# bbc/turingcodec

Hardware: AMD Instinct MI355X
Metric: encoded fps (havoc hot path, primitive-batch throughput: one picture's primitive calls per frame as whole-frame batches; (higher is better)
Workload: dtype u8; 1 GPU; 1920x1080 8-bit 4:2:0 random-access QP32 speed=medium B-frame, MEASURED call mix of the reference encoder on this clip generator (profiles/r04_reference_call_mi; calls_per_frame=3944815, launches_per_frame=49, pictures_in_flight=2, parallelism=single GPU

## Files before the change

include/havoc_mi355x.h:

```cpp
#ifndef HAVOC_MI355X_H
#define HAVOC_MI355X_H

#include <stddef.h>
#include <stdint.h>

#ifdef __cplusplus
extern "C" {
#endif

#define HAVOC_MI355X_EINVAL (-10001)
#define HAVOC_MI355X_ENODEV (-10002)
#define HAVOC_MI355X_EDEVICE (-10003)

typedef struct havoc_mi355x_ctx havoc_mi355x_ctx;

#define HAVOC_MI355X_NEW_STREAM ((void *)(intptr_t)-1)
int havoc_mi355x_create(havoc_mi355x_ctx **ctx, int device, void *stream);
void havoc_mi355x_destroy(havoc_mi355x_ctx *ctx);
int havoc_mi355x_set_stream(havoc_mi355x_ctx *ctx, void *stream);
int havoc_mi355x_sync(havoc_mi355x_ctx *ctx);
int havoc_mi355x_sync_spin(havoc_mi355x_ctx *ctx);
const char *havoc_mi355x_last_error(void);
const char *havoc_mi355x_version(void);
int havoc_mi355x_device_info(havoc_mi355x_ctx *ctx, int64_t info[8]);
// ... 92 lines not shown
typedef struct {
    int32_t dst_off, src_off;
    int32_t n;
    int32_t scale, shift, offset;
    int32_t reserved[2];
} havoc_mi355x_quant_job;


int havoc_mi355x_pad_block(havoc_mi355x_ctx *ctx, int S, void *d_plane, int64_t origin_off, int width, int height,
                           intptr_t stride, int pad, int top, int bottom, int left, int right);

int havoc_mi355x_deblock(havoc_mi355x_ctx *ctx, int S, int bitDepth, void *d_luma, intptr_t stride_luma, void *d_cb, void *d_cr, intptr_t stride_chroma,
                         int width, int height, const int8_t *d_block_data, const uint8_t *d_block_bs, int tc_offset_div2, int beta_offset_div2,
                         int cb_qp_offset, int cr_qp_offset);

typedef struct {
    int16_t mv[2][2];
    int8_t dpb_index[2];
    uint8_t flags;
    int8_t qp_y;
    uint8_t tu_log2;
    uint8_t reserved[3];
} havoc_mi355x_cell;
enum {
    HAVOC_CELL_INTRA = 1,
    HAVOC_CELL_CODED = 2,
    HAVOC_CELL_NO_FILTER = 4,
    HAVOC_CELL_PU_LEFT = 8,
    HAVOC_CELL_PU_TOP = 16
};
int havoc_mi355x_derive_bs(havoc_mi355x_ctx *ctx, const havoc_mi355x_cell *d_cells, intptr_t cells_stride, int width, int height, int8_t *d_block_data,
                           uint8_t *d_block_bs);

typedef struct havoc_mi355x_picture havoc_mi355x_picture;
int havoc_mi355x_picture_create(havoc_mi355x_ctx *ctx, int S, int bit_depth, int width, int height, int pad, int alignment,
                                havoc_mi355x_picture **pic);
void havoc_mi355x_picture_destroy(havoc_mi355x_ctx *ctx, havoc_mi355x_picture *pic);
int havoc_mi355x_picture_plane(havoc_mi355x_picture *pic, int cIdx, void **d_base, int64_t *origin_off, intptr_t *stride, int *width, int *height,
                               int *pad);
int havoc_mi355x_picture_upload_yuv(havoc_mi355x_ctx *ctx, havoc_mi355x_picture *pic, const void *h_yuv, int src_S, int shift, int pad_after);
int havoc_mi355x_picture_upload_plane(havoc_mi355x_ctx *ctx, havoc_mi355x_picture *pic, int cIdx, const void *h_origin, intptr_t h_stride,
                                      int with_padding);
int havoc_mi355x_picture_download_plane(havoc_mi355x_ctx *ctx, havoc_mi355x_picture *pic, int cIdx, void *h_origin, intptr_t h_stride,
                                        int with_padding);
int havoc_mi355x_picture_pad(havoc_mi355x_ctx *ctx, havoc_mi355x_picture *pic);
int havoc_mi355x_picture_phase_planes(havoc_mi355x_ctx *ctx, havoc_mi355x_picture *pic, void **d_planes, intptr_t *plane_elems, int64_t *luma_first);


int havoc_mi355x_sad(havoc_mi355x_ctx *ctx, int S, const void *d_src, intptr_t stride_src, const void *d_ref,
                     intptr_t stride_ref, const havoc_mi355x_pair_job *d_jobs, int njobs, int32_t *d_out);
int havoc_mi355x_sad4(havoc_mi355x_ctx *ctx, int S, const void *d_src, intptr_t stride_src, const void *d_ref,
                      intptr_t stride_ref, const havoc_mi355x_sad4_job *d_jobs, int njobs, int32_t *d_out);
typedef struct {
    int32_t first_job;
    int32_t count;
    int32_t box_off, box_w, box_h;
    int32_t reserved[3];
} havoc_mi355x_sad4_run;
int havoc_mi355x_sad4_runs(havoc_mi355x_ctx *ctx, int S, const void *d_src, intptr_t stride_src, const void *d_ref,
                           intptr_t stride_ref, const havoc_mi355x_sad4_job *d_jobs, int njobs,
                           const havoc_mi355x_sad4_run *d_runs, int nruns, int32_t *d_out);
int havoc_mi355x_sad4_make_runs(const havoc_mi355x_sad4_job *jobs, int njobs, int max_run, intptr_t stride_ref, int S, havoc_mi355x_sad4_run *runs);
int havoc_mi355x_sad_surface(havoc_mi355x_ctx *ctx, int S, int range, int max_w, int max_h, const void *d_src,
                             intptr_t stride_src, const void *d_ref, intptr_t stride_ref,
                             const havoc_mi355x_surface_job *d_jobs, int njobs, int32_t *d_out);
int havoc_mi355x_ssd(havoc_mi355x_ctx *ctx, int S, const void *d_a, intptr_t stride_a, const void *d_b,
                     intptr_t stride_b, const havoc_mi355x_pair_job *d_jobs, int njobs, uint32_t *d_out);
int havoc_mi355x_satd(havoc_mi355x_ctx *ctx, int S, int max_w, int max_h, const void *d_a, intptr_t stride_a, const void *d_b,
                      intptr_t stride_b, const havoc_mi355x_pair_job *d_jobs, int njobs, int32_t *d_out);
int havoc_mi355x_satd_multi(havoc_mi355x_ctx *ctx, int S, int max_w, int max_h, const void *d_a, intptr_t stride_a,
                            const void *d_b, intptr_t stride_b, const havoc_mi355x_satd_multi_job *d_jobs, int njobs,
                            int32_t *d_out);
int havoc_mi355x_ssd_linear(havoc_mi355x_ctx *ctx, const uint8_t *d_a, const uint8_t *d_b, int size, int32_t *d_out);


int havoc_mi355x_pred_uni(havoc_mi355x_ctx *ctx, int S, int taps, int bitDepth, int max_w, int max_h, void *d_dst, intptr_t stride_dst,
                          const void *d_ref, intptr_t stride_ref, const havoc_mi355x_pred_uni_job *d_jobs, int njobs);
int havoc_mi355x_pred_bi(havoc_mi355x_ctx *ctx, int S, int taps, int bitDepth, int max_w, int max_h, void *d_dst, intptr_t stride_dst,
                         const void *d_ref, intptr_t stride_ref, const havoc_mi355x_pred_bi_job *d_jobs, int njobs);
int havoc_mi355x_pred_uni_classes(havoc_mi355x_ctx *ctx, int S, int taps, int bitDepth, void *d_dst, intptr_t stride_dst, const void *d_ref,
                                  intptr_t stride_ref, const havoc_mi355x_pred_uni_job *d_jobs, const int32_t count[4]);
int havoc_mi355x_pred_bi_classes(havoc_mi355x_ctx *ctx, int S, int taps, int bitDepth, void *d_dst, intptr_t stride_dst, const void *d_ref,
                                 intptr_t stride_ref, const havoc_mi355x_pred_bi_job *d_jobs, const int32_t count[4]);
int havoc_mi355x_subtract_bi(havoc_mi355x_ctx *ctx, int S, int bitDepth, void *d_dst, intptr_t stride_dst,
                             const void *d_pred, intptr_t stride_pred, const void *d_src, intptr_t stride_src,
                             const havoc_mi355x_subtract_bi_job *d_jobs, int njobs);

int havoc_mi355x_interp_planes(havoc_mi355x_ctx *ctx, int S, int bitDepth, void *d_planes, intptr_t plane_elems, const void *d_ref,
                               intptr_t stride, int x0, int y0, int width, int height);

int havoc_mi355x_subpel_satd(havoc_mi355x_ctx *ctx, int S, int taps, int bitDepth, int max_w, int max_h, const void *d_src,
                             intptr_t stride_src, const void *d_ref, intptr_t stride_ref, const havoc_mi355x_pred_uni_job *d_jobs,
                             int njobs, int32_t *d_cost);


int havoc_mi355x_intra(havoc_mi355x_ctx *ctx, int S, int bitDepth, int log2TrafoSize, void *d_dst, intptr_t stride_dst,
                       const void *d_neighbours, const havoc_mi355x_intra_job *d_jobs, int njobs);

typedef struct {
    int32_t src_off;
    int32_t nb_off;
    int32_t nbf_off;
    uint32_t filt_lo;
    uint32_t filt_hi;
    int32_t edge;
    int32_t reserved[2];
} havoc_mi355x_intra_search_job;
int havoc_mi355x_intra_satd35(havoc_mi355x_ctx *ctx, int S, int bitDepth, int log2TrafoSize, const void *d_src, intptr_t stride_src,
                              const void *d_neighbours, const havoc_mi355x_intra_search_job *d_jobs, int njobs, int32_t *d_cost);


int havoc_mi355x_residual(havoc_mi355x_ctx *ctx, int S, int16_t *d_res, intptr_t stride_res, const int32_t *d_res_off,
                          const void *d_src, intptr_t stride_src, const void *d_pred, intptr_t stride_pred,
                          const havoc_mi355x_pair_job *d_jobs, int njobs);
int havoc_mi355x_transform(havoc_mi355x_ctx *ctx, int bitDepth, int trType, int log2TrafoSize, int16_t *d_coeffs,
                           const int16_t *d_res, intptr_t stride_res, const havoc_mi355x_tu_job *d_jobs, int njobs);
int havoc_mi355x_inverse_transform(havoc_mi355x_ctx *ctx, int bitDepth, int trType, int log2TrafoSize, int16_t *d_res,
                                   const int16_t *d_coeffs, const havoc_mi355x_tu_job *d_jobs, int njobs);
int havoc_mi355x_inverse_transform_add(havoc_mi355x_ctx *ctx, int S, int bitDepth, int trType, int log2TrafoSize,
                                       void *d_dst, intptr_t stride_dst, const void *d_pred, intptr_t stride_pred,
                                       const int16_t *d_coeffs, const havoc_mi355x_tu_job *d_jobs, int njobs);
typedef struct {
    int32_t coef_off;
    int32_t src_off;
    int32_t pred_off;
    int32_t rec_off;
} havoc_mi355x_tu_fused_job;
int havoc_mi355x_tu_forward(havoc_mi355x_ctx *ctx, int S, int bitDepth, int trType, int log2TrafoSize, int16_t *d_coeffs, const void *d_src,
                            intptr_t stride_src, const void *d_pred, intptr_t stride_pred, const havoc_mi355x_tu_fused_job *d_jobs, int njobs);
int havoc_mi355x_intra_measure(havoc_mi355x_ctx *ctx, int S, int bitDepth, int log2TrafoSize, int16_t *d_coeffs, int16_t *d_coeffs_dct, int32_t *d_satd, void *d_rec0,
                               uint32_t *d_ssd0, const void *d_src, intptr_t stride_src, const void *d_pred, intptr_t stride_pred, const havoc_mi355x_tu_fused_job *d_jobs,
                               int njobs, int with_satd);
int havoc_mi355x_tu_reconstruct(havoc_mi355x_ctx *ctx, int S, int bitDepth, int trType, int log2TrafoSize, int scale, int shift, void *d_rec,
                                intptr_t stride_rec, const void *d_pred, intptr_t stride_pred, const void *d_src, intptr_t stride_src,
                                const int16_t *d_levels, const havoc_mi355x_tu_fused_job *d_jobs, int njobs, uint32_t *d_ssd);

int havoc_mi355x_level_stats(havoc_mi355x_ctx *ctx, const int16_t *d_levels, const int32_t *d_jobs, int njobs, int32_t *d_out);

int havoc_mi355x_quantize(havoc_mi355x_ctx *ctx, int16_t *d_dst, const int16_t *d_src,
                          const havoc_mi355x_quant_job *d_jobs, int njobs, int32_t *d_cbf);
int havoc_mi355x_quantize_inverse(havoc_mi355x_ctx *ctx, int16_t *d_dst, const int16_t *d_src,
                                  const havoc_mi355x_quant_job *d_jobs, int njobs);
int havoc_mi355x_quantize_reconstruct(havoc_mi355x_ctx *ctx, int log2TrafoSize, uint8_t *d_rec, intptr_t stride_rec,
                                      const uint8_t *d_pred, intptr_t stride_pred, const int16_t *d_res,
                                      const havoc_mi355x_tu_job *d_jobs, int njobs);

typedef struct {
    int32_t src_off, rec_off;
    int32_t w, h;
} havoc_mi355x_sao_stats_job;
int havoc_mi355x_sao_stats(havoc_mi355x_ctx *ctx, int S, int bitDepth, const void *d_src, intptr_t stride_src, const void *d_rec, intptr_t stride_rec,
                           const havoc_mi355x_sao_stats_job *d_jobs, int njobs, int64_t *d_out);
typedef struct {
    int32_t src_u, src_v;
    int32_t rec_u, rec_v;
    int32_t w, h;
    int32_t reserved[2];
} havoc_mi355x_sao_chroma_job;
int havoc_mi355x_sao_band_chroma(havoc_mi355x_ctx *ctx, int S, int bitDepth, const void *d_src, intptr_t stride_src, const void *d_rec, intptr_t stride_rec,
                                 const havoc_mi355x_sao_chroma_job *d_jobs, int njobs, int64_t *d_out);
typedef struct {
    int32_t dst_off, src_off, w, h;
    int32_t type, eo_class;
    int16_t offsets[32];
    int32_t reserved[2];
} havoc_mi355x_sao_job;
// ... 439 lines not shown
```

turingcodec_amd/csrc/api.hip:

```cpp
#include "common.h"
#include "launch.h"

#include <cstdio>
#include <cstring>
#include <initializer_list>

using namespace havoc_gpu;

static_assert(sizeof(havoc_mi355x_pair_job) == 16, "job ABI");
static_assert(sizeof(havoc_mi355x_sad4_job) == 32, "job ABI");
static_assert(sizeof(havoc_mi355x_surface_job) == 32, "job ABI");
static_assert(sizeof(havoc_mi355x_satd_multi_job) == 80, "job ABI");
static_assert(sizeof(havoc_mi355x_pred_uni_job) == 32, "job ABI");
static_assert(sizeof(havoc_mi355x_pred_bi_job) == 48, "job ABI");
static_assert(sizeof(havoc_mi355x_subtract_bi_job) == 32, "job ABI");
static_assert(sizeof(havoc_mi355x_intra_job) == 32, "job ABI");
static_assert(sizeof(havoc_mi355x_tu_job) == 16, "job ABI");
static_assert(sizeof(havoc_mi355x_intra_search_job) == 32, "job ABI");
static_assert(sizeof(havoc_mi355x_tu_fused_job) == 16, "job ABI");
static_assert(sizeof(havoc_mi355x_quant_job) == 32, "job ABI");
static_assert(sizeof(havoc_mi355x_sao_ctu) == 64 && sizeof(havoc_mi355x_sao_component) == 44 && sizeof(havoc_mi355x_sao_params) == 128 && sizeof(havoc_mi355x_sao_bounds) == 32,
              "sao record ABI");
static_assert(offsetof(havoc_mi355x_sao_params, dist_sao) == 88 && offsetof(havoc_mi355x_sao_params, ssd_sao) == 96 && offsetof(havoc_mi355x_sao_ctu, stat_src_cb) == 48,
              "sao record ABI");
// ... 396 lines not shown
{
    REQUIRE_CTX(); REQUIRE_S(); REQUIRE(njobs >= 0, "njobs < 0");
    REQUIRE(max_w >= 2 && max_w <= 64 && max_h >= 2 && max_h <= 64, "max_w / max_h must be 2..64");
    return check(launch_satd(LS(ctx),S, max_w, max_h, d_a, stride_a, d_b, stride_b, d_jobs, njobs, d_out), "satd");
}

int havoc_mi355x_satd_multi(havoc_mi355x_ctx *ctx, int S, int max_w, int max_h, const void *d_a, intptr_t stride_a, const void *d_b,
                            intptr_t stride_b, const havoc_mi355x_satd_multi_job *d_jobs, int njobs, int32_t *d_out)
{
    REQUIRE_CTX(); REQUIRE_S(); REQUIRE(njobs >= 0, "njobs < 0");
    REQUIRE(max_w >= 2 && max_w <= 64 && max_h >= 2 && max_h <= 64, "max_w / max_h must be 2..64");
    return check(launch_satd_multi(LS(ctx), S, max_w, max_h, d_a, stride_a, d_b, stride_b, d_jobs, njobs, d_out), "satd_multi");
}

int havoc_mi355x_pad_block(havoc_mi355x_ctx *ctx, int S, void *d_plane, int64_t origin_off, int width, int height, intptr_t stride, int pad, int top,
                           int bottom, int left, int right)
{
    REQUIRE_CTX(); REQUIRE_S();
    REQUIRE(width > 0 && height > 0 && pad >= 0, "width / height must be positive, pad >= 0");
    return check(launch_pad_block(LS(ctx), S, d_plane, (long)origin_off, width, height, stride, pad, top, bottom, left, right), "pad_block");
}

int havoc_mi355x_derive_bs(havoc_mi355x_ctx *ctx, const havoc_mi355x_cell *d_cells, intptr_t cells_stride, int width, int height, int8_t *d_block_data,
                           uint8_t *d_block_bs)
{
    REQUIRE_CTX();
    REQUIRE(d_cells && d_block_data && d_block_bs, "null pointer");
    REQUIRE(width > 0 && height > 0 && (width & 7) == 0 && (height & 7) == 0 && cells_stride >= width / 4, "picture size must be a multiple of 8 (minimum coding unit)");
    return check(launch_derive_bs(LS(ctx), d_cells, (long)cells_stride, width, height, d_block_data, d_block_bs), "derive_bs");
}

int havoc_mi355x_deblock(havoc_mi355x_ctx *ctx, int S, int bitDepth, void *d_luma, intptr_t stride_luma, void *d_cb, void *d_cr, intptr_t stride_chroma,
                         int width, int height, const int8_t *d_block_data, const uint8_t *d_block_bs, int tc_offset_div2, int beta_offset_div2,
                         int cb_qp_offset, int cr_qp_offset)
{
    REQUIRE_CTX(); REQUIRE_S(); REQUIRE_BD();
    REQUIRE(width >= 8 && height >= 8 && (width & 7) == 0 && (height & 7) == 0, "width / height must be multiples of 8 (minimum coding block)");
    REQUIRE(d_luma && d_cb && d_cr && d_block_data && d_block_bs, "null plane / block map");
    REQUIRE(tc_offset_div2 >= -6 && tc_offset_div2 <= 6 && beta_offset_div2 >= -6 && beta_offset_div2 <= 6, "slice offsets must be -6..6");
    return check(launch_deblock(LS(ctx), S, bitDepth, d_luma, stride_luma, d_cb, d_cr, stride_chroma, width, height, d_block_data, d_block_bs,
                                tc_offset_div2, beta_offset_div2, cb_qp_offset, cr_qp_offset),
                 "deblock");
}

int havoc_mi355x_ssd_linear(havoc_mi355x_ctx *ctx, const uint8_t *d_a, const uint8_t *d_b, int size, int32_t *d_out)
{
    REQUIRE_CTX(); REQUIRE(size >= 0, "size < 0");
    return check(launch_ssd_linear(LS(ctx),d_a, d_b, size, d_out), "ssd_linear");
}


#define REQUIRE_MAXWH() REQUIRE(max_w >= 2 && max_w <= 64 && max_h >= 2 && max_h <= 64, "max_w / max_h must be 2..64")

int havoc_mi355x_pred_uni(havoc_mi355x_ctx *ctx, int S, int taps, int bitDepth, int max_w, int max_h, void *d_dst, intptr_t stride_dst,
                          const void *d_ref, intptr_t stride_ref, const havoc_mi355x_pred_uni_job *d_jobs, int njobs)
{
    REQUIRE_CTX(); REQUIRE_S(); REQUIRE_BD(); REQUIRE(taps == 8 || taps == 4, "taps must be 8 or 4"); REQUIRE(njobs >= 0, "njobs < 0");
    REQUIRE_MAXWH();
    return check(launch_pred_uni(LS(ctx),S, taps, bitDepth, max_w, max_h, d_dst, stride_dst, d_ref, stride_ref, d_jobs, njobs), "pred_uni");
}

int havoc_mi355x_pred_bi(havoc_mi355x_ctx *ctx, int S, int taps, int bitDepth, int max_w, int max_h, void *d_dst, intptr_t stride_dst,
                         const void *d_ref, intptr_t stride_ref, const havoc_mi355x_pred_bi_job *d_jobs, int njobs)
{
    REQUIRE_CTX(); REQUIRE_S(); REQUIRE_BD(); REQUIRE(taps == 8 || taps == 4, "taps must be 8 or 4"); REQUIRE(njobs >= 0, "njobs < 0");
    REQUIRE_MAXWH();
    return check(launch_pred_bi(LS(ctx),S, taps, bitDepth, max_w, max_h, d_dst, stride_dst, d_ref, stride_ref, d_jobs, njobs), "pred_bi");
}

int havoc_mi355x_pred_uni_classes(havoc_mi355x_ctx *ctx, int S, int taps, int bitDepth, void *d_dst, intptr_t stride_dst, const void *d_ref, intptr_t stride_ref,
                                  const havoc_mi355x_pred_uni_job *d_jobs, const int32_t count[4])
{
    REQUIRE_CTX(); REQUIRE_S(); REQUIRE_BD(); REQUIRE(taps == 8 || taps == 4, "taps must be 8 or 4"); REQUIRE(count != nullptr, "null count");
    return check(launch_pred_uni_classes(LS(ctx), S, taps, bitDepth, d_dst, stride_dst, d_ref, stride_ref, d_jobs, count), "pred_uni_classes");
}

int havoc_mi355x_pred_bi_classes(havoc_mi355x_ctx *ctx, int S, int taps, int bitDepth, void *d_dst, intptr_t stride_dst, const void *d_ref, intptr_t stride_ref,
                                 const havoc_mi355x_pred_bi_job *d_jobs, const int32_t count[4])
{
    REQUIRE_CTX(); REQUIRE_S(); REQUIRE_BD(); REQUIRE(taps == 8 || taps == 4, "taps must be 8 or 4"); REQUIRE(count != nullptr, "null count");
    return check(launch_pred_bi_classes(LS(ctx), S, taps, bitDepth, d_dst, stride_dst, d_ref, stride_ref, d_jobs, count), "pred_bi_classes");
}

int havoc_mi355x_subtract_bi(havoc_mi355x_ctx *ctx, int S, int bitDepth, void *d_dst, intptr_t stride_dst, const void *d_pred, intptr_t stride_pred,
                             const void *d_src, intptr_t stride_src, const havoc_mi355x_subtract_bi_job *d_jobs, int njobs)
{
    REQUIRE_CTX(); REQUIRE_S(); REQUIRE_BD(); REQUIRE(njobs >= 0, "njobs < 0");
    return check(launch_subtract_bi(LS(ctx),S, bitDepth, d_dst, stride_dst, d_pred, stride_pred, d_src, stride_src, d_jobs, njobs), "subtract_bi");
}

int havoc_mi355x_interp_planes(havoc_mi355x_ctx *ctx, int S, int bitDepth, void *d_planes, intptr_t plane_elems, const void *d_ref, intptr_t stride,
                               int x0, int y0, int width, int height)
{
    REQUIRE_CTX(); REQUIRE_S(); REQUIRE_BD(); REQUIRE(x0 >= 3 && y0 >= 3 && width >= 0 && height >= 0, "rectangle must start >= 3 samples in");
    REQUIRE(x0 + width + 12 <= stride, "rectangle must end >= 12 samples before the row end");
    return check(launch_interp_planes(LS(ctx), S, bitDepth, d_planes, plane_elems, d_ref, stride, x0, y0, width, height), "interp_planes");
}

int havoc_mi355x_subpel_satd(havoc_mi355x_ctx *ctx, int S, int taps, int bitDepth, int max_w, int max_h, const void *d_src, intptr_t stride_src,
                             const void *d_ref, intptr_t stride_ref, const havoc_mi355x_pred_uni_job *d_jobs, int njobs, int32_t *d_cost)
{
    REQUIRE_CTX(); REQUIRE_S(); REQUIRE_BD(); REQUIRE(taps == 8 || taps == 4, "taps must be 8 or 4"); REQUIRE(njobs >= 0, "njobs < 0");
    REQUIRE(max_w >= 2 && max_w <= 64 && max_h >= 2 && max_h <= 64, "max_w / max_h must be 2..64");
    return check(launch_subpel_satd(LS(ctx),S, taps, bitDepth, max_w, max_h, d_src, stride_src, d_ref, stride_ref, d_jobs, njobs, d_cost),
                 "subpel_satd");
}


int havoc_mi355x_intra(havoc_mi355x_ctx *ctx, int S, int bitDepth, int log2TrafoSize, void *d_dst, intptr_t stride_dst, const void *d_neighbours,
                       const havoc_mi355x_intra_job *d_jobs, int njobs)
{
    REQUIRE_CTX(); REQUIRE_S(); REQUIRE_BD(); REQUIRE(log2TrafoSize >= 2 && log2TrafoSize <= 5, "log2TrafoSize must be 2..5");
    REQUIRE(njobs >= 0, "njobs < 0");
    return check(launch_intra(LS(ctx),S, log2TrafoSize, bitDepth, d_dst, stride_dst, d_neighbours, d_jobs, njobs), "intra");
}

int havoc_mi355x_intra_satd35(havoc_mi355x_ctx *ctx, int S, int bitDepth, int log2TrafoSize, const void *d_src, intptr_t stride_src,
                              const void *d_neighbours, const havoc_mi355x_intra_search_job *d_jobs, int njobs, int32_t *d_cost)
{
    REQUIRE_CTX(); REQUIRE_S(); REQUIRE_BD(); REQUIRE(log2TrafoSize >= 2 && log2TrafoSize <= 5, "log2TrafoSize must be 2..5");
    REQUIRE(njobs >= 0, "njobs < 0");
    return check(launch_intra_satd35(LS(ctx),S, log2TrafoSize, bitDepth, d_src, stride_src, d_neighbours, d_jobs, njobs, d_cost), "intra_satd35");
}


int havoc_mi355x_residual(havoc_mi355x_ctx *ctx, int S, int16_t *d_res, intptr_t stride_res, const int32_t *d_res_off, const void *d_src,
                          intptr_t stride_src, const void *d_pred, intptr_t stride_pred, const havoc_mi355x_pair_job *d_jobs, int njobs)
{
    REQUIRE_CTX(); REQUIRE_S(); REQUIRE(njobs >= 0, "njobs < 0");
    return check(launch_residual(LS(ctx),S, d_res, stride_res, d_res_off, d_src, stride_src, d_pred, stride_pred, d_jobs, njobs), "residual");
}

#define REQUIRE_TR() \
    REQUIRE(log2TrafoSize >= 2 && log2TrafoSize <= 5, "log2TrafoSize must be 2..5"); \
    REQUIRE(trType == 0 || (trType == 1 && log2TrafoSize == 2), "trType 1 (DST) requires log2TrafoSize 2")

int havoc_mi355x_transform(havoc_mi355x_ctx *ctx, int bitDepth, int trType, int log2TrafoSize, int16_t *d_coeffs, const int16_t *d_res,
                           intptr_t stride_res, const havoc_mi355x_tu_job *d_jobs, int njobs)
{
    REQUIRE_CTX(); REQUIRE_TR(); REQUIRE(bitDepth >= 8 && bitDepth <= 10, "bitDepth must be 8..10"); REQUIRE(njobs >= 0, "njobs < 0");
    return check(launch_transform(LS(ctx),bitDepth, log2TrafoSize, trType, d_coeffs, d_res, stride_res, d_jobs, njobs), "transform");
}

int havoc_mi355x_inverse_transform(havoc_mi355x_ctx *ctx, int bitDepth, int trType, int log2TrafoSize, int16_t *d_res, const int16_t *d_coeffs,
                                   const havoc_mi355x_tu_job *d_jobs, int njobs)
{
    REQUIRE_CTX(); REQUIRE_TR(); REQUIRE(bitDepth >= 8 && bitDepth <= 10, "bitDepth must be 8..10"); REQUIRE(njobs >= 0, "njobs < 0");
    return check(launch_inverse_transform(LS(ctx),0, bitDepth, log2TrafoSize, trType, nullptr, 0, nullptr, 0, d_res, d_coeffs, d_jobs, njobs),
                 "inverse_transform");
}

int havoc_mi355x_inverse_transform_add(havoc_mi355x_ctx *ctx, int S, int bitDepth, int trType, int log2TrafoSize, void *d_dst, intptr_t stride_dst,
                                       const void *d_pred, intptr_t stride_pred, const int16_t *d_coeffs, const havoc_mi355x_tu_job *d_jobs,
                                       int njobs)
{
    REQUIRE_CTX(); REQUIRE_S(); REQUIRE_BD(); REQUIRE_TR(); REQUIRE(njobs >= 0, "njobs < 0");
    return check(launch_inverse_transform(LS(ctx),S, bitDepth, log2TrafoSize, trType, d_dst, stride_dst, d_pred, stride_pred, nullptr, d_coeffs,
                                          d_jobs, njobs),
                 "inverse_transform_add");
}

int havoc_mi355x_tu_forward(havoc_mi355x_ctx *ctx, int S, int bitDepth, int trType, int log2TrafoSize, int16_t *d_coeffs, const void *d_src,
                            intptr_t stride_src, const void *d_pred, intptr_t stride_pred, const havoc_mi355x_tu_fused_job *d_jobs, int njobs)
{
    REQUIRE_CTX(); REQUIRE_S(); REQUIRE_BD(); REQUIRE_TR(); REQUIRE(njobs >= 0, "njobs < 0");
    return check(launch_tu_forward(LS(ctx), S, bitDepth, log2TrafoSize, trType, d_coeffs, d_src, stride_src, d_pred, stride_pred, d_jobs, njobs),
// ... 724 lines not shown
```

turingcodec_amd/csrc/kernels_inter.hip:

```cpp
#include <stdlib.h>

#include "common.h"
#include "launch.h"
#include "interp.h"

namespace havoc_gpu {

template <int MAXW, int MAXH, int G, bool BI>
struct PredLds
{
    static constexpr int JPW = 256 / G, NREF = BI ? 2 : 1, TH = MAXH + 8, OS = MAXW + 2;
    static constexpr int tmpElems = MAXW * TH + 8, outElems = MAXH * OS + 2;
    static constexpr int tmpBytes = ((JPW * NREF * tmpElems * 2) + 15) & ~15;
    static constexpr int bytes = tmpBytes + ((JPW * outElems * 2 + 15) & ~15);
};

template <int S, int TAPS, int MAXW, int MAXH, int G, bool BI>
__device__ __forceinline__ void pred_workgroup_full(char *lds, char *__restrict__ dst, long stride_dst, const char *__restrict__ ref, long stride_ref,
                                                    const int32_t *__restrict__ jobs, int njobs, int bitDepth, int wg, int wgs)
{
    typedef typename Sample<S>::T T;
    typedef PredLds<MAXW, MAXH, G, BI> L;
    constexpr int JPW = 256 / G;
    constexpr int NREF = BI ? 2 : 1;
    constexpr int AB = TAPS / 2 - 1;
    constexpr int TH = MAXH + 8;
    constexpr int OS = MAXW + 2;
    int16_t (*s_tmp)[NREF][L::tmpElems] = reinterpret_cast<int16_t (*)[NREF][L::tmpElems]>(lds);
    uint16_t (*s_out)[L::outElems] = reinterpret_cast<uint16_t (*)[L::outElems]>(lds + L::tmpBytes);

    const int sub = threadIdx.x / G, l = threadIdx.x - sub * G;
    const int job = xcd_block(wg, wgs) * JPW + sub;
    const bool live = job < njobs;
    const int32_t *j = jobs + (long)(live ? job : 0) * (BI ? 12 : 8);
    const int w = BI ? j[3] : j[2], h = BI ? j[4] : j[3];
    const long dsb = stride_dst * S, rsb = stride_ref * S;
    const int maxv = (1 << bitDepth) - 1;
    const int shift1 = min(4, bitDepth - 8);
    const int shift3 = max(2, 14 - bitDepth);
    const int qpr = (w + 3) >> 2, wh = h + TAPS - 1;
    const FastDiv fq(qpr);

#pragma unroll
    for (int r = 0; r < NREF; ++r)
    {
        const char *r0 = ref + (long)j[1 + r] * S;
        int cx[TAPS];
        taps_of<TAPS>(BI ? j[5 + 2 * r] : j[4], cx);
        int16_t *tmp = s_tmp[sub][r];
        for (int i = l; i < wh * qpr; i += G)
        {
            const int y = fq.div(i), x0 = (i - y * qpr) * 4;
            int a[4];
            hfilter4<S, TAPS>(r0 + (y - AB) * rsb + (x0 - AB) * S, cx, a);
#pragma unroll
            for (int o = 0; o < 4; ++o)
                if (x0 + o < w) tmp[(x0 + o) * TH + y] = (int16_t)(a[o] >> shift1);
        }
    }
    __syncthreads();

    {
        uint32_t cp[NREF][TAPS / 2];
#pragma unroll
        for (int r = 0; r < NREF; ++r)
        {
            int cy[TAPS];
            taps_of<TAPS>(BI ? j[6 + 2 * r] : j[5], cy);
#pragma unroll
            for (int k = 0; k < TAPS / 2; ++k) cp[r][k] = pack_i16(cy[2 * k], cy[2 * k + 1]);
        }
        const int groups = (h + 7) >> 3;
        const FastDiv fw(w);
        uint16_t *ot = s_out[sub];
        for (int it = l; it < (live ? w * groups : 0); it += G)
        {
            const int gy = fw.div(it), x = it - gy * w;
            const int y0 = gy * 8;
            int acc[8];
#pragma unroll
            for (int r = 0; r < NREF; ++r)
            {
                const int16_t *col = &s_tmp[sub][r][x * TH + y0];
                const u32x4 q0 = *reinterpret_cast<const u32x4 *>(col), q1 = *reinterpret_cast<const u32x4 *>(col + 8);
                const uint32_t e[8] = {q0.x, q0.y, q0.z, q0.w, q1.x, q1.y, q1.z, q1.w};
                uint32_t od[7];
#pragma unroll
                for (int k = 0; k < 7; ++k) od[k] = __builtin_amdgcn_alignbit(e[k + 1], e[k], 16);
#pragma unroll
                for (int jj = 0; jj < 8; ++jj)
                {
                    int a = 0;
#pragma unroll
                    for (int k = 0; k < TAPS / 2; ++k) a = sdot2((jj & 1) ? od[(jj >> 1) + k] : e[(jj >> 1) + k], cp[r][k], a);
                    if (!BI) acc[jj] = a;
                    else if (r == 0) acc[jj] = a >> 6;
                    else acc[jj] += a >> 6;
                }
            }
#pragma unroll
            for (int jj = 0; jj < 8; ++jj)
            {
                const int v = BI ? (acc[jj] + (1 << shift3)) >> (shift3 + 1) : (acc[jj] + (1 << (5 + shift3))) >> (6 + shift3);
                if (y0 + jj < h) ot[(y0 + jj) * OS + x] = (uint16_t)clip3(0, maxv, v);
            }
        }
    }
    __syncthreads();

    if (!live) return;
    char *d = dst + (long)j[0] * S;
    const uint16_t *ot = s_out[sub];
    for (int i = l; i < h * qpr; i += G)
    {
        const int y = fq.div(i), x0 = (i - y * qpr) * 4;
        const uint16_t *p = ot + y * OS + x0;
        char *q = d + y * dsb + x0 * S;
        if (x0 + 4 <= w)
        {
            if (S == 1) st4(q, (uint32_t)p[0] | ((uint32_t)p[1] << 8) | ((uint32_t)p[2] << 16) | ((uint32_t)p[3] << 24));
            else st8(q, u32x2{(uint32_t)p[0] | ((uint32_t)p[1] << 16), (uint32_t)p[2] | ((uint32_t)p[3] << 16)});
        }
        else
            for (int o = 0; x0 + o < w; ++o) reinterpret_cast<T *>(q)[o] = (T)p[o];
    }
}


template <int MAXW, int MAXH, int G, bool BI>
struct PredLeanLds
{
    static constexpr int JPW = 256 / G, NREF = BI ? 2 : 1, TH = MAXH + 8, QSKEW = 8;
    static constexpr int tileElems = MAXW * TH + (MAXW / 4) * QSKEW;
    static constexpr int bytes = JPW * NREF * tileElems * 2;
    static_assert(bytes <= PredLds<MAXW, MAXH, G, BI>::bytes, "the lean form lives in the full form's LDS");
};

constexpr int kDppXor2 = 0x4E;

template <int S>
__device__ __forceinline__ void store_quad_rows(char *q, long dsb, const int (&v)[8], int c, int rowsLeft)
{
    if (S == 1)
    {
        const uint32_t selA = (c & 1) ? 0x03070105u : 0x06020400u, selB = (c & 2) ? 0x03020706u : 0x05040100u;
#pragma unroll
        for (int half = 0; half < 2; ++half)
        {
            const int *u = v + 4 * half;
            uint32_t d = (uint32_t)u[0] | ((uint32_t)u[1] << 8) | ((uint32_t)u[2] << 16) | ((uint32_t)u[3] << 24);
            d = __builtin_amdgcn_perm((uint32_t)dpp_mov<kDppXor1>((int)d), d, selA);
            d = __builtin_amdgcn_perm((uint32_t)dpp_mov<kDppXor2>((int)d), d, selB);
            if (c + 4 * half < rowsLeft) st4(q + 4 * half * dsb, d);
        }
    }
    else
    {
        const uint32_t selA = (c & 1) ? 0x03020706u : 0x05040100u;
        const bool hi = (c & 2) != 0;
#pragma unroll
        for (int half = 0; half < 2; ++half)
        {
            const int *u = v + 4 * half;
            uint32_t e0 = (uint32_t)u[0] | ((uint32_t)u[1] << 16), e1 = (uint32_t)u[2] | ((uint32_t)u[3] << 16);
            e0 = __builtin_amdgcn_perm((uint32_t)dpp_mov<kDppXor1>((int)e0), e0, selA);
            e1 = __builtin_amdgcn_perm((uint32_t)dpp_mov<kDppXor1>((int)e1), e1, selA);
            const uint32_t t = (uint32_t)dpp_mov<kDppXor2>((int)(hi ? e0 : e1));
            if (c + 4 * half < rowsLeft) st8(q + 4 * half * dsb, u32x2{hi ? t : e0, hi ? e1 : t});
        }
    }
}

template <int JPW, bool BI>
__device__ __forceinline__ bool widths_are_quads(const int32_t *__restrict__ jobs, int njobs, int wg, int wgs)
{
    const int lane = threadIdx.x & (kWave - 1);
    const int job = xcd_block(wg, wgs) * JPW + lane;
    int w = 0;
    if (lane < JPW && job < njobs) w = jobs[(long)job * (BI ? 12 : 8) + (BI ? 3 : 2)];
    return __ballot(w & 3) == 0;
}

template <int S, int TAPS, int MAXW, int MAXH, int G, bool BI>
__device__ __forceinline__ void pred_workgroup_lean(char *lds, char *__restrict__ dst, long stride_dst, const char *__restrict__ ref, long stride_ref,
                                                    const int32_t *__restrict__ jobs, int njobs, int bitDepth, int wg, int wgs)
{
    typedef PredLeanLds<MAXW, MAXH, G, BI> L;
    constexpr int JPW = 256 / G;
    constexpr int NREF = BI ? 2 : 1;
    constexpr int AB = TAPS / 2 - 1;
    constexpr int TH = L::TH;
    constexpr bool ZP = G >= kWave;
    int16_t *s_tile = reinterpret_cast<int16_t *>(lds);

    const int sub = ZP ? __builtin_amdgcn_readfirstlane((int)threadIdx.x / G) : (int)threadIdx.x / G;
    const int l = threadIdx.x - sub * G;
    const int job = xcd_block(wg, wgs) * JPW + sub;
    const bool live = job < njobs;
    const int32_t *j = jobs + (long)(live ? job : 0) * (BI ? 12 : 8);
    const int w = BI ? j[3] : j[2], h = BI ? j[4] : j[3];
    const long dsb = stride_dst * S, rsb = stride_ref * S;
    const int maxv = (1 << bitDepth) - 1;
    const int shift1 = min(4, bitDepth - 8);
    const int shift3 = max(2, 14 - bitDepth);
    const int qpr = w >> 2, wh = h + TAPS - 1;

    {
        const FastDiv fq(qpr);
        const int rp0 = fq.div(l), q = l - rp0 * qpr, rstep = fq.div(G);
        if (live && rp0 < rstep)
        {
#pragma unroll
            for (int r = 0; r < NREF; ++r)
            {
                const int xf = BI ? j[5 + 2 * r] : j[4], yf = BI ? j[6 + 2 * r] : j[5];
                const bool xz = ZP && xf == 0, yz = ZP && yf == 0;
                const int rows = yz ? h : wh;
                const char *p = ref + ((long)j[1 + r] + q * 4) * S + (long)(2 * rp0 - (yz ? 0 : AB)) * rsb;
                const long step = 2L * rstep * rsb;
                uint32_t *cw = reinterpret_cast<uint32_t *>(s_tile + (sub * NREF + r) * L::tileElems + q * (4 * TH + L::QSKEW)) + rp0;
                if (xz)
                {
                    const int sh = 6 - shift1;
                    for (int y = 2 * rp0; y < rows; y += 2 * rstep, p += step, cw += rstep)
                    {
                        const char *p1 = p + (y + 1 < rows ? rsb : 0);
                        if (S == 1)
                        {
                            const uint32_t a = ld4(p), b = ld4(p1);
#pragma unroll
                            for (int o = 0; o < 4; ++o) cw[o * (TH / 2)] = __builtin_amdgcn_perm(b, a, 0x0c000c00u | ((4u + o) << 16) | o) << sh;
                        }
                        else
                        {
                            const u32x2 a = ld8(p), b = ld8(p1);
                            cw[0 * (TH / 2)] = __builtin_amdgcn_perm(b.x, a.x, 0x05040100u) << sh;
                            cw[1 * (TH / 2)] = __builtin_amdgcn_perm(b.x, a.x, 0x07060302u) << sh;
                            cw[2 * (TH / 2)] = __builtin_amdgcn_perm(b.y, a.y, 0x05040100u) << sh;
                            cw[3 * (TH / 2)] = __builtin_amdgcn_perm(b.y, a.y, 0x07060302u) << sh;
                        }
                    }
                }
                else
                {
                    int cx[TAPS];
                    taps_of<TAPS>(xf, cx);
                    p -= AB * S;
                    for (int y = 2 * rp0; y < rows; y += 2 * rstep, p += step, cw += rstep)
                    {
                        HRaw<S, TAPS> ra, rb;
                        hfilter4_load<S, TAPS>(p, ra);
                        hfilter4_load<S, TAPS>(p + (y + 1 < rows ? rsb : 0), rb);
                        int a[4], b[4];
                        hfilter4_eval<S, TAPS>(ra, cx, a);
                        hfilter4_eval<S, TAPS>(rb, cx, b);
#pragma unroll
                        for (int o = 0; o < 4; ++o)
                            cw[o * (TH / 2)] = __builtin_amdgcn_perm((uint32_t)(b[o] >> shift1), (uint32_t)(a[o] >> shift1), 0x05040100u);
                    }
                }
            }
        }
    }
    __syncthreads();
    if (!live) return;

    uint32_t cp[NREF][TAPS / 2];
    bool yz[NREF];
#pragma unroll
    for (int r = 0; r < NREF; ++r)
    {
        const int yf = BI ? j[6 + 2 * r] : j[5];
        yz[r] = ZP && yf == 0;
        int cy[TAPS];
        taps_of<TAPS>(yf, cy);
#pragma unroll
        for (int k = 0; k < TAPS / 2; ++k) cp[r][k] = pack_i16(cy[2 * k], cy[2 * k + 1]);
    }
    const int groups = (h + 7) >> 3;
    const FastDiv fw(w);
    char *d = dst + (long)j[0] * S;
    const int c = l & 3;
    for (int it = l; it < w * groups; it += G)
    {
        const int gy = fw.div(it), x = it - gy * w;
        const int y0 = gy * 8;
        int acc[8];
#pragma unroll
        for (int r = 0; r < NREF; ++r)
        {
            const int16_t *col = s_tile + (sub * NREF + r) * L::tileElems + x * TH + (x >> 2) * L::QSKEW + y0;
            const u32x4 q0 = *reinterpret_cast<const u32x4 *>(col);
            if (yz[r])
            {
                const uint32_t e[4] = {q0.x, q0.y, q0.z, q0.w};
#pragma unroll
                for (int jj = 0; jj < 8; ++jj)
                {
                    const int t = (jj & 1) ? (int)e[jj >> 1] >> 16 : (int)(e[jj >> 1] << 16) >> 16;
                    if (!BI) acc[jj] = t * 64;
                    else if (r == 0) acc[jj] = t;
                    else acc[jj] += t;
                }
            }
            else
            {
                const u32x4 q1 = *reinterpret_cast<const u32x4 *>(col + 8);
                const uint32_t e[8] = {q0.x, q0.y, q0.z, q0.w, q1.x, q1.y, q1.z, q1.w};
                uint32_t od[7];
#pragma unroll
                for (int k = 0; k < 7; ++k) od[k] = __builtin_amdgcn_alignbit(e[k + 1], e[k], 16);
#pragma unroll
                for (int jj = 0; jj < 8; ++jj)
                {
                    int a = 0;
#pragma unroll
                    for (int k = 0; k < TAPS / 2; ++k) a = sdot2((jj & 1) ? od[(jj >> 1) + k] : e[(jj >> 1) + k], cp[r][k], a);
                    if (!BI) acc[jj] = a;
                    else if (r == 0) acc[jj] = a >> 6;
                    else acc[jj] += a >> 6;
                }
            }
        }
#pragma unroll
        for (int jj = 0; jj < 8; ++jj)
        {
            const int v = BI ? (acc[jj] + (1 << shift3)) >> (shift3 + 1) : (acc[jj] + (1 << (5 + shift3))) >> (6 + shift3);
            acc[jj] = clip3(0, maxv, v);
        }
        store_quad_rows<S>(d + (y0 + c) * dsb + (x - c) * S, dsb, acc, c, h - y0);
    }
}

template <int S, int TAPS, int MAXW, int MAXH, int G, bool BI>
__device__ __forceinline__ void pred_workgroup(char *lds, char *__restrict__ dst, long stride_dst, const char *__restrict__ ref, long stride_ref,
                                               const int32_t *__restrict__ jobs, int njobs, int bitDepth, int wg, int wgs, int lean)
{
    if (lean && widths_are_quads<256 / G, BI>(jobs, njobs, wg, wgs))
        pred_workgroup_lean<S, TAPS, MAXW, MAXH, G, BI>(lds, dst, stride_dst, ref, stride_ref, jobs, njobs, bitDepth, wg, wgs);
    else
        pred_workgroup_full<S, TAPS, MAXW, MAXH, G, BI>(lds, dst, stride_dst, ref, stride_ref, jobs, njobs, bitDepth, wg, wgs);
}

template <int S, int TAPS, int MAXW, int MAXH, int G, bool BI>
__global__ __launch_bounds__(256) void k_pred(char *__restrict__ dst, long stride_dst, const char *__restrict__ ref, long stride_ref,
                                              const int32_t *__restrict__ jobs, int njobs, int bitDepth, int lean)
{
    __shared__ __attribute__((aligned(16))) char lds[PredLds<MAXW, MAXH, G, BI>::bytes];
    pred_workgroup<S, TAPS, MAXW, MAXH, G, BI>(lds, dst, stride_dst, ref, stride_ref, jobs, njobs, bitDepth, blockIdx.x, gridDim.x, lean);
}

struct PredClasses { int count[4], firstWg[5]; };

template <int S, int TAPS, bool BI>
__global__ __launch_bounds__(256) void k_pred_classes(char *__restrict__ dst, long stride_dst, const char *__restrict__ ref, long stride_ref,
                                                      const int32_t *__restrict__ jobs, PredClasses pc, int bitDepth, int lean)
{
    __shared__ __attribute__((aligned(16))) char lds[PredLds<64, 64, 256, BI>::bytes];
    constexpr int words = BI ? 12 : 8;
    const int wg = blockIdx.x;
    if (wg < pc.firstWg[1])
        pred_workgroup<S, TAPS, 8, 8, 8, BI>(lds, dst, stride_dst, ref, stride_ref, jobs, pc.count[0], bitDepth, wg, pc.firstWg[1], lean);
    else if (wg < pc.firstWg[2])
        pred_workgroup<S, TAPS, 16, 16, 32, BI>(lds, dst, stride_dst, ref, stride_ref, jobs + (long)pc.count[0] * words, pc.count[1], bitDepth, wg - pc.firstWg[1],
                                                pc.firstWg[2] - pc.firstWg[1], lean);
    else if (wg < pc.firstWg[3])
        pred_workgroup<S, TAPS, 32, 32, 128, BI>(lds, dst, stride_dst, ref, stride_ref, jobs + (long)(pc.count[0] + pc.count[1]) * words, pc.count[2], bitDepth,
                                                 wg - pc.firstWg[2], pc.firstWg[3] - pc.firstWg[2], lean);
    else
        pred_workgroup<S, TAPS, 64, 64, 256, BI>(lds, dst, stride_dst, ref, stride_ref, jobs + (long)(pc.count[0] + pc.count[1] + pc.count[2]) * words, pc.count[3],
                                                 bitDepth, wg - pc.firstWg[3], pc.firstWg[4] - pc.firstWg[3], lean);
}

template <int S>
__global__ __launch_bounds__(256) void k_subtract_bi(char *__restrict__ dst, long stride_dst, const char *__restrict__ pred, long stride_pred,
                                                     const char *__restrict__ src, long stride_src, const int32_t *__restrict__ jobs, int njobs,
                                                     int bitDepth, int lean)
{
    typedef typename Sample<S>::T T;
    const int job = xcd_block(blockIdx.x, gridDim.x) * 4 + __builtin_amdgcn_readfirstlane((int)threadIdx.x >> 6);
    const int lane = threadIdx.x & 63;
    if (job >= njobs) return;
    const int32_t *j = jobs + job * 8;
    const int w = j[3], h = j[4];
    T *d = reinterpret_cast<T *>(dst) + j[0];
    const T *p = reinterpret_cast<const T *>(pred) + j[1];
    const T *s = reinterpret_cast<const T *>(src) + j[2];
    const int maxv = (1 << bitDepth) - 1;
    if (lean && (w & 3) == 0 && w <= 4 * kWave)
    {
        const int qpr = w >> 2;
        const FastDiv fq(qpr);
        const int y0 = fq.div(lane), q = lane - y0 * qpr, ystep = fq.div(kWave);
        if (y0 >= ystep) return;
        const long db = stride_dst * S, pb = stride_pred * S, sb = stride_src * S;
        char *dd = reinterpret_cast<char *>(d + 4 * q) + y0 * db;
        const char *pp = reinterpret_cast<const char *>(p + 4 * q) + y0 * pb, *ss = reinterpret_cast<const char *>(s + 4 * q) + y0 * sb;
        const s16x2 zero = {0, 0}, top = {(short)maxv, (short)maxv};
        auto sub_clip = [&](uint32_t sv, uint32_t pv) {
            const s16x2 a = __builtin_bit_cast(s16x2, sv), b = __builtin_bit_cast(s16x2, pv);
            return __builtin_bit_cast(uint32_t, __builtin_elementwise_min(__builtin_elementwise_max(a + a - b, zero), top));
        };
        for (int y = y0; y < h; y += ystep, dd += ystep * db, pp += ystep * pb, ss += ystep * sb)
        {
            if (S == 1)
            {
                const uint32_t sv = ld4(ss), pv = ld4(pp);
                const uint32_t lo = sub_clip(__builtin_amdgcn_perm(0u, sv, 0x0c010c00u), __builtin_amdgcn_perm(0u, pv, 0x0c010c00u));
                const uint32_t hi = sub_clip(__builtin_amdgcn_perm(0u, sv, 0x0c030c02u), __builtin_amdgcn_perm(0u, pv, 0x0c030c02u));
                st4(dd, __builtin_amdgcn_perm(hi, lo, 0x06040200u));
            }
            else
            {
                const u32x2 sv = ld8(ss), pv = ld8(pp);
                st8(dd, u32x2{sub_clip(sv.x, pv.x), sub_clip(sv.y, pv.y)});
            }
        }
        return;
    }
    const FastDiv fd(w);
    for (int i = lane; i < w * h; i += kWave)
    {
        const int y = fd.div(i), x = i - y * w;
        d[y * stride_dst + x] = (T)clip3(0, maxv, 2 * (int)s[y * stride_src + x] - (int)p[y * stride_pred + x]);
    }
}

static int pred_lean()
{
    static const int on = !(getenv("HAVOC_PRED_LEAN") && atoi(getenv("HAVOC_PRED_LEAN")) == 0);
    return on;
}

template <int S, int TAPS, bool BI>
static hipError_t launch_pred_st(hipStream_t st, int bd, int maxw, int maxh, char *dst, long sd, const char *ref, long sr, const int32_t *jobs, int n)
{
    const dim3 b(256);
    if (maxw <= 8 && maxh <= 8)
        hipLaunchKernelGGL((k_pred<S, TAPS, 8, 8, 8, BI>), dim3((n + 31) / 32), b, 0, st, dst, sd, ref, sr, jobs, n, bd, pred_lean());
    else if (maxw <= 16 && maxh <= 16)
        hipLaunchKernelGGL((k_pred<S, TAPS, 16, 16, 32, BI>), dim3((n + 7) / 8), b, 0, st, dst, sd, ref, sr, jobs, n, bd, pred_lean());
    else if (maxw <= 32 && maxh <= 32)
        hipLaunchKernelGGL((k_pred<S, TAPS, 32, 32, 128, BI>), dim3((n + 1) / 2), b, 0, st, dst, sd, ref, sr, jobs, n, bd, pred_lean());
    else
        hipLaunchKernelGGL((k_pred<S, TAPS, 64, 64, 256, BI>), dim3(n), b, 0, st, dst, sd, ref, sr, jobs, n, bd, pred_lean());
    return hipGetLastError();
}

template <bool BI>
static hipError_t launch_pred(hipStream_t st, int S, int taps, int bd, int maxw, int maxh, void *dst, long sd, const void *ref, long sr,
                              const int32_t *j, int n)
{
    if (n <= 0) return hipSuccess;
    char *d = (char *)dst;
    const char *r = (const char *)ref;
    if (S == 1 && taps == 8) return launch_pred_st<1, 8, BI>(st, bd, maxw, maxh, d, sd, r, sr, j, n);
    if (S == 1 && taps == 4) return launch_pred_st<1, 4, BI>(st, bd, maxw, maxh, d, sd, r, sr, j, n);
    if (S == 2 && taps == 8) return launch_pred_st<2, 8, BI>(st, bd, maxw, maxh, d, sd, r, sr, j, n);
    if (S == 2 && taps == 4) return launch_pred_st<2, 4, BI>(st, bd, maxw, maxh, d, sd, r, sr, j, n);
    return hipErrorInvalidValue;
}

hipError_t launch_pred_uni(hipStream_t st, int S, int taps, int bd, int maxw, int maxh, void *dst, long sd, const void *ref, long sr,
                           const havoc_mi355x_pred_uni_job *jobs, int n)
{
    return launch_pred<false>(st, S, taps, bd, maxw, maxh, dst, sd, ref, sr, (const int32_t *)jobs, n);
}

hipError_t launch_pred_bi(hipStream_t st, int S, int taps, int bd, int maxw, int maxh, void *dst, long sd, const void *ref, long sr,
                          const havoc_mi355x_pred_bi_job *jobs, int n)
{
    return launch_pred<true>(st, S, taps, bd, maxw, maxh, dst, sd, ref, sr, (const int32_t *)jobs, n);
}

template <bool BI>
static hipError_t launch_pred_classes_t(hipStream_t st, int S, int taps, int bd, void *dst, long sd, const void *ref, long sr, const int32_t *j, const int count[4])
{
    PredClasses pc;
    static const int jpw[4] = {32, 8, 2, 1};
    pc.firstWg[0] = 0;
    for (int c = 0; c < 4; ++c)
    {
        if (count[c] < 0) return hipErrorInvalidValue;
        pc.count[c] = count[c];
        pc.firstWg[c + 1] = pc.firstWg[c] + (count[c] + jpw[c] - 1) / jpw[c];
    }
    if (pc.firstWg[4] == 0) return hipSuccess;
    char *d = (char *)dst;
    const char *r = (const char *)ref;
    const dim3 g(pc.firstWg[4]), b(256);
    if (S == 1 && taps == 8) hipLaunchKernelGGL((k_pred_classes<1, 8, BI>), g, b, 0, st, d, sd, r, sr, j, pc, bd, pred_lean());
    else if (S == 1 && taps == 4) hipLaunchKernelGGL((k_pred_classes<1, 4, BI>), g, b, 0, st, d, sd, r, sr, j, pc, bd, pred_lean());
    else if (S == 2 && taps == 8) hipLaunchKernelGGL((k_pred_classes<2, 8, BI>), g, b, 0, st, d, sd, r, sr, j, pc, bd, pred_lean());
    else if (S == 2 && taps == 4) hipLaunchKernelGGL((k_pred_classes<2, 4, BI>), g, b, 0, st, d, sd, r, sr, j, pc, bd, pred_lean());
    else return hipErrorInvalidValue;
    return hipGetLastError();
}

hipError_t launch_pred_bi_classes(hipStream_t st, int S, int taps, int bd, void *dst, long sd, const void *ref, long sr, const havoc_mi355x_pred_bi_job *jobs, const int count[4])
{
    return launch_pred_classes_t<true>(st, S, taps, bd, dst, sd, ref, sr, (const int32_t *)jobs, count);
}

hipError_t launch_pred_uni_classes(hipStream_t st, int S, int taps, int bd, void *dst, long sd, const void *ref, long sr, const havoc_mi355x_pred_uni_job *jobs, const int count[4])
{
    return launch_pred_classes_t<false>(st, S, taps, bd, dst, sd, ref, sr, (const int32_t *)jobs, count);
}

hipError_t launch_subtract_bi(hipStream_t st, int S, int bitDepth, void *dst, long sd, const void *pred, long sp, const void *src, long ss,
                              const havoc_mi355x_subtract_bi_job *jobs, int n)
{
    if (n <= 0) return hipSuccess;
    if (S == 1)
        hipLaunchKernelGGL((k_subtract_bi<1>), dim3((n + 3) / 4), dim3(256), 0, st, (char *)dst, sd, (const char *)pred, sp, (const char *)src, ss,
                           (const int32_t *)jobs, n, bitDepth, pred_lean());
    else
        hipLaunchKernelGGL((k_subtract_bi<2>), dim3((n + 3) / 4), dim3(256), 0, st, (char *)dst, sd, (const char *)pred, sp, (const char *)src, ss,
                           (const int32_t *)jobs, n, bitDepth, pred_lean());
    return hipGetLastError();
}

}
```

turingcodec_amd/csrc/kernels_metric.hip:

```cpp
#include "common.h"
#include "launch.h"

#include <cstdlib>

namespace havoc_gpu {


template <int S>
__device__ __forceinline__ uint32_t sad_dword(uint32_t a, uint32_t b, uint32_t acc)
{
    if (S == 1) return __builtin_amdgcn_sad_u8(a, b, acc);
    return __builtin_amdgcn_sad_u16(a, b, acc);
}

#ifndef SADL
#define SADL 16
#endif
constexpr int kSadLanes = SADL;
__device__ __forceinline__ int sad_group_sum(int v)
{
    v += __builtin_amdgcn_update_dpp(0, v, 0x111, 0xf, 0xf, true);
    v += __builtin_amdgcn_update_dpp(0, v, 0x112, 0xf, 0xf, true);
    v += __builtin_amdgcn_update_dpp(0, v, 0x114, 0xf, 0xe, true);
    if (kSadLanes == 16) v += __builtin_amdgcn_update_dpp(0, v, 0x118, 0xf, 0xc, true);
    return v;
}

__device__ __forceinline__ int smallDiv(int x, int c) { return (int)(((float)x + 0.5f) * __builtin_amdgcn_rcpf((float)c)); }
__device__ __forceinline__ int mul24(int a, int b) { return __mul24(a, b); }
__device__ __forceinline__ uint32_t mulu24(uint32_t a, uint32_t b) { return __umul24(a, b); }

template <int S, int WAYS, int CB, int U = 4>
__device__ __forceinline__ void sad_block(const char *src, long ssb, const char *const (&ref)[WAYS], long rsb, int rowBytes, int h,
                                          int lane, uint32_t (&acc)[WAYS])
{
    const int cpr = rowBytes / CB;
    const int rpi = smallDiv(kSadLanes, cpr);
    const int y0 = smallDiv(lane, cpr);
    const int xb = (lane - y0 * cpr) * CB;
    if (y0 >= rpi) return;
#pragma unroll U
    for (int y = y0; y < h; y += rpi)
    {
        const char *s = src + y * ssb + xb;
        if (CB == 4)
        {
            const uint32_t a = ld4(s);
#pragma unroll
            for (int k = 0; k < WAYS; ++k) acc[k] = sad_dword<S>(a, ld4(ref[k] + y * rsb + xb), acc[k]);
        }
        else if (CB == 8)
        {
            const u32x2 a = ld8(s);
#pragma unroll
            for (int k = 0; k < WAYS; ++k)
            {
                const u32x2 b = ld8(ref[k] + y * rsb + xb);
                acc[k] = sad_dword<S>(a.x, b.x, acc[k]);
                acc[k] = sad_dword<S>(a.y, b.y, acc[k]);
            }
        }
        else
        {
            const u32x4 a = ld16(s);
#pragma unroll
            for (int k = 0; k < WAYS; ++k)
            {
                const u32x4 b = ld16(ref[k] + y * rsb + xb);
                acc[k] = sad_dword<S>(a.x, b.x, acc[k]);
                acc[k] = sad_dword<S>(a.y, b.y, acc[k]);
                acc[k] = sad_dword<S>(a.z, b.z, acc[k]);
                acc[k] = sad_dword<S>(a.w, b.w, acc[k]);
            }
        }
    }
}

template <int S, int WAYS, int U = 4, int MINW = 1>
__global__ __launch_bounds__(256, MINW) void k_sad(const char *__restrict__ src, long stride_src, const char *__restrict__ ref, long stride_ref,
                                             const int32_t *__restrict__ jobs, int njobs, int32_t *__restrict__ out)
{
    typedef typename Sample<S>::T T;
    const int job = (xcd_block(blockIdx.x, gridDim.x) * 256 + threadIdx.x) / kSadLanes;
    const int lane = threadIdx.x & (kSadLanes - 1);
// ... 646 lines not shown
        int total[4];
        sad4_job<S, kFallWB>(src, stride_src, ref, stride_ref, inv_stride_ref, j0 + (long)(live ? c : 0) * 8, live, &lds[group * kFallD], lane, total);
        if (live && lane == kSadLanes - 1)
#pragma unroll
            for (int k = 0; k < 4; ++k) out[((long)first + c) * 4 + k] = total[k];
    }
}

template <int S, int NW, int U, bool SRCG = true>
__global__ __launch_bounds__(64 * NW) void k_sad4r(const char *__restrict__ src, long stride_src, const char *__restrict__ ref, long stride_ref, float inv_stride_ref,
                                                   const int32_t *__restrict__ jobs, int njobs, const int32_t *__restrict__ runs, int nruns, int32_t *__restrict__ out)
{
    __shared__ RunLds<S> sh;
    sad4_run_general<S, NW, U, SRCG>(sh, src, stride_src, ref, stride_ref, inv_stride_ref, jobs, njobs, runs, xcd_block(blockIdx.x, gridDim.x), out);
}


template <int S, int CB>
__device__ __forceinline__ uint32_t ssd_block(const char *a, long sab, const char *b, long sbb, int rowBytes, int h, int lane)
{
    const int cpr = rowBytes / CB;
    const int rpi = kSadLanes / cpr;
    const int y0 = lane / cpr;
    const int xb = (lane - y0 * cpr) * CB;
    uint32_t acc = 0;
    if (y0 >= rpi) return 0;
#pragma unroll 2
    for (int y = y0; y < h; y += rpi)
    {
        const char *p = a + y * sab + xb, *q = b + y * sbb + xb;
        if (CB == 4) acc = ssd_dword<S>(ld4(p), ld4(q), acc);
        else if (CB == 8)
        {
            const u32x2 u = ld8(p), v = ld8(q);
            acc = ssd_dword<S>(u.x, v.x, acc);
            acc = ssd_dword<S>(u.y, v.y, acc);
        }
        else
        {
            const u32x4 u = ld16(p), v = ld16(q);
            acc = ssd_dword<S>(u.x, v.x, acc);
            acc = ssd_dword<S>(u.y, v.y, acc);
            acc = ssd_dword<S>(u.z, v.z, acc);
            acc = ssd_dword<S>(u.w, v.w, acc);
        }
    }
    return acc;
}

template <int S>
__global__ __launch_bounds__(256) void k_ssd(const char *__restrict__ pa, long stride_a, const char *__restrict__ pb, long stride_b,
                                             const int32_t *__restrict__ jobs, int njobs, uint32_t *__restrict__ out)
{
    typedef typename Sample<S>::T T;
    const int job = (xcd_block(blockIdx.x, gridDim.x) * 256 + threadIdx.x) / kSadLanes;
    const int lane = threadIdx.x & (kSadLanes - 1);
    const bool live = job < njobs;
    const int32_t *j = jobs + (long)(live ? job : 0) * 4;
    const int w = j[2], h = live ? j[3] : 0;
    const long sab = stride_a * S, sbb = stride_b * S;
    const char *a = pa + (long)j[0] * S;
    const char *b = pb + (long)j[1] * S;
    uint32_t acc = 0;
    const int rowBytes = w * S;
    if ((rowBytes & 15) == 0 && rowBytes <= 16 * kSadLanes) acc = ssd_block<S, 16>(a, sab, b, sbb, rowBytes, h, lane);
    else if ((rowBytes & 7) == 0 && rowBytes <= 8 * kSadLanes) acc = ssd_block<S, 8>(a, sab, b, sbb, rowBytes, h, lane);
    else if ((rowBytes & 3) == 0 && rowBytes <= 4 * kSadLanes) acc = ssd_block<S, 4>(a, sab, b, sbb, rowBytes, h, lane);
    else
    {
        const FastDiv fd(w);
        for (int i = lane; i < w * h; i += kSadLanes)
        {
            const int y = fd.div(i), x = i - y * w;
            const int d = (int)reinterpret_cast<const T *>(a + y * sab)[x] - (int)reinterpret_cast<const T *>(b + y * sbb)[x];
            acc += (uint32_t)(d * d);
        }
    }
    uint32_t t = (uint32_t)sad_group_sum((int)acc);
    if (S == 2) t >>= 4;
    if (live && lane == kSadLanes - 1) out[job] = t;
}


template <int S, int N>
__device__ __forceinline__ void load_diff_row(const char *a, const char *b, int (&d)[N])
{
    if (S == 1)
    {
        if (N == 8)
        {
            const u32x2 va = ld8(a), vb = ld8(b);
#pragma unroll
            for (int x = 0; x < 4; ++x)
            {
                d[x] = (int)((va.x >> (8 * x)) & 0xff) - (int)((vb.x >> (8 * x)) & 0xff);
                d[x + 4] = (int)((va.y >> (8 * x)) & 0xff) - (int)((vb.y >> (8 * x)) & 0xff);
            }
        }
        else
        {
            const uint32_t va = ld4(a), vb = ld4(b);
#pragma unroll
            for (int x = 0; x < 4; ++x) d[x] = (int)((va >> (8 * x)) & 0xff) - (int)((vb >> (8 * x)) & 0xff);
        }
    }
    else
    {
        if (N == 8)
        {
            const u32x4 va = ld16(a), vb = ld16(b);
            const uint32_t wa[4] = {va.x, va.y, va.z, va.w}, wb[4] = {vb.x, vb.y, vb.z, vb.w};
#pragma unroll
            for (int x = 0; x < 4; ++x)
            {
                d[2 * x] = (int)(wa[x] & 0xffff) - (int)(wb[x] & 0xffff);
                d[2 * x + 1] = (int)(wa[x] >> 16) - (int)(wb[x] >> 16);
            }
        }
        else
        {
            const u32x2 va = ld8(a), vb = ld8(b);
            d[0] = (int)(va.x & 0xffff) - (int)(vb.x & 0xffff);
            d[1] = (int)(va.x >> 16) - (int)(vb.x >> 16);
            d[2] = (int)(va.y & 0xffff) - (int)(vb.y & 0xffff);
            d[3] = (int)(va.y >> 16) - (int)(vb.y >> 16);
        }
    }
}

template <int S, int G>
__global__ __launch_bounds__(256) void k_satd(const char *__restrict__ pa, long stride_a, const char *__restrict__ pb, long stride_b,
                                              const int32_t *__restrict__ jobs, int njobs, int32_t *__restrict__ out)
{
    typedef typename Sample<S>::T T;
    const int job = (xcd_block(blockIdx.x, gridDim.x) * 256 + threadIdx.x) / G;
    const int l = threadIdx.x & (G - 1);
    const bool live = job < njobs;
    const int32_t *j = jobs + (long)(live ? job : 0) * 4;
    const int w = j[2], h = live ? j[3] : 0;
    const long sab = stride_a * S, sbb = stride_b * S;
    const char *a = pa + (long)j[0] * S;
    const char *b = pb + (long)j[1] * S;
    int acc = 0;
    if (((w | h) & 7) == 0)
    {
        const int tw = w >> 3;
        const FastDiv fd(tw);
        for (int it = l; it < tw * (h >> 3) * 8; it += G)
        {
            const int tile = it >> 3, r = it & 7;
            const int ty = fd.div(tile), tx = tile - ty * tw;
            const char *pa8 = a + (long)(ty * 8 + r) * sab + tx * 8 * S, *pb8 = b + (long)(ty * 8 + r) * sbb + tx * 8 * S;
            if (S == 1)
            {
                const u32x2 va = ld8(pa8), vb = ld8(pb8);
                const uint32_t m = 0x00ff00ffu;
                uint32_t p[4] = {pk_sub(va.x & m, vb.x & m), pk_sub((va.x >> 8) & m, (vb.x >> 8) & m),
                                 pk_sub(va.y & m, vb.y & m), pk_sub((va.y >> 8) & m, (vb.y >> 8) & m)};
                acc += satd_rows_pk<8>(p, r);
            }
            else
            {
                int d[8];
                load_diff_row<S, 8>(pa8, pb8, d);
                acc += satd_rows<S, 8>(d, r);
            }
        }
    }
    else if (((w | h) & 3) == 0)
    {
        const int tw = w >> 2;
        const FastDiv fd(tw);
        for (int it = l; it < tw * (h >> 2) * 4; it += G)
        {
            const int tile = it >> 2, r = it & 3;
            const int ty = fd.div(tile), tx = tile - ty * tw;
            const char *pa4 = a + (long)(ty * 4 + r) * sab + tx * 4 * S, *pb4 = b + (long)(ty * 4 + r) * sbb + tx * 4 * S;
            if (S == 1)
            {
                const uint32_t va = ld4(pa4), vb = ld4(pb4), m = 0x00ff00ffu;
                uint32_t p[2] = {pk_sub(va & m, vb & m), pk_sub((va >> 8) & m, (vb >> 8) & m)};
                acc += satd_rows_pk<4>(p, r);
            }
            else
            {
                int d[4];
                load_diff_row<S, 4>(pa4, pb4, d);
                acc += satd_rows<S, 4>(d, r);
            }
        }
    }
    else
    {
        const int tw = w >> 1;
        const FastDiv fd(tw);
        for (int t = l; t < tw * (h >> 1); t += G)
        {
            const int ty = fd.div(t), tx = t - ty * tw;
            const T *p = reinterpret_cast<const T *>(a + (long)(2 * ty) * sab) + 2 * tx;
            const T *q = reinterpret_cast<const T *>(b + (long)(2 * ty) * sbb) + 2 * tx;
            const int d0 = (int)p[0] - (int)q[0], d1 = (int)p[1] - (int)q[1];
            const int d2 = (int)p[stride_a] - (int)q[stride_b], d3 = (int)p[stride_a + 1] - (int)q[stride_b + 1];
            int sum = abs(d0 + d1 + d2 + d3) + abs(d0 - d1 + d2 - d3) + abs(d0 + d1 - d2 - d3) + abs(d0 - d1 - d2 + d3);
            if (S == 2) sum >>= 2;
            acc += sum;
        }
    }
    const int t = G == 64 ? wave_sum(acc) : group_sum<G>(acc);
    if (live && l == 0) out[job] = t;
}

constexpr int kSatdMulti = 16;

template <int S, int G, int CPS, bool TILE = false>
__global__ __launch_bounds__(256) void k_satd_multi(const char *__restrict__ pa, long stride_a, const char *__restrict__ pb, long stride_b,
                                                    const int32_t *__restrict__ jobs, int njobs, int32_t *__restrict__ out)
{
    typedef typename Sample<S>::T T;
    constexpr int SL = kSatdMulti / CPS;
    const int grp = (xcd_block(blockIdx.x, gridDim.x) * 256 + threadIdx.x) / G;
    const int job = grp / SL, k0 = (grp - job * SL) * CPS;
    const int l = threadIdx.x & (G - 1);
    const bool live = job < njobs;
    const int32_t *j = jobs + (long)(live ? job : 0) * (4 + kSatdMulti);
    const int w = j[1], cnt = min(max(j[3], 0), kSatdMulti), h = (live && k0 < cnt) ? j[2] : 0;
    const long sab = stride_a * S, sbb = stride_b * S;
    const char *a = pa + (long)j[0] * S;
    const char *b[CPS];
#pragma unroll
    for (int k = 0; k < CPS; ++k) b[k] = pb + (long)j[4 + max(0, min(k0 + k, cnt - 1))] * S;
    int acc[CPS];
#pragma unroll
    for (int k = 0; k < CPS; ++k) acc[k] = 0;
    if (TILE && S == 2 && ((w | h) & 7) == 0)
    {
        const int tw = w >> 3;
        const FastDiv fd(tw);
        for (int t = l; t < tw * (h >> 3); t += G)
        {
            const int ty = fd.div(t), tx = t - ty * tw;
            const char *pa8 = a + (long)(ty * 8) * sab + tx * 16;
            const long ob = (long)(ty * 8) * sbb + tx * 16;
            uint32_t ap[8][4];
#pragma unroll
            for (int r = 0; r < 8; ++r)
            {
                const u32x4 va = ld16(pa8 + r * sab);
                ap[r][0] = va.x; ap[r][1] = va.y; ap[r][2] = va.z; ap[r][3] = va.w;
            }
#pragma unroll
            for (int k = 0; k < CPS; ++k)
            {
                uint32_t d[8][4];
#pragma unroll
                for (int r = 0; r < 8; ++r)
                {
                    const u32x4 vb = ld16(b[k] + ob + r * sbb);
                    d[r][0] = pk_sub(ap[r][0], vb.x); d[r][1] = pk_sub(ap[r][1], vb.y); d[r][2] = pk_sub(ap[r][2], vb.z); d[r][3] = pk_sub(ap[r][3], vb.w);
                }
                acc[k] += satd_tile8_pk16(d);
            }
        }
    }
    else if (TILE && S == 1 && ((w | h) & 7) == 0)
    {
        const int tw = w >> 3;
        const FastDiv fd(tw);
        const uint32_t m = 0x00ff00ffu;
        for (int t = l; t < tw * (h >> 3); t += G)
        {
            const int ty = fd.div(t), tx = t - ty * tw;
            const char *pa8 = a + (long)(ty * 8) * sab + tx * 8;
            const long ob = (long)(ty * 8) * sbb + tx * 8;
            uint32_t ap[8][4];
#pragma unroll
            for (int r = 0; r < 8; ++r)
            {
                const u32x2 va = ld8(pa8 + r * sab);
                ap[r][0] = va.x & m; ap[r][1] = (va.x >> 8) & m; ap[r][2] = va.y & m; ap[r][3] = (va.y >> 8) & m;
            }
#pragma unroll
            for (int k = 0; k < CPS; ++k)
            {
                uint32_t d[8][4];
#pragma unroll
                for (int r = 0; r < 8; ++r)
                {
                    const u32x2 vb = ld8(b[k] + ob + r * sbb);
                    d[r][0] = pk_sub(ap[r][0], vb.x & m); d[r][1] = pk_sub(ap[r][1], (vb.x >> 8) & m);
                    d[r][2] = pk_sub(ap[r][2], vb.y & m); d[r][3] = pk_sub(ap[r][3], (vb.y >> 8) & m);
// ... 264 lines not shown
```

turingcodec_amd/csrc/launch.h:

```cpp
#pragma once

#include "common.h"

namespace havoc_gpu {
hipError_t launch_sad(hipStream_t, int S, const void *, long, const void *, long, const havoc_mi355x_pair_job *, int, int32_t *);
hipError_t launch_sad4(hipStream_t, int S, const void *, long, const void *, long, const havoc_mi355x_sad4_job *, int, int32_t *);
hipError_t launch_sad4_runs(hipStream_t, int S, const void *, long, const void *, long, const havoc_mi355x_sad4_job *, int, const havoc_mi355x_sad4_run *, int, int32_t *);
hipError_t launch_sad_surface(hipStream_t, int S, int range, int maxw, int maxh, const void *, long, const void *, long, const havoc_mi355x_surface_job *, int, int32_t *);
hipError_t launch_ssd(hipStream_t, int S, const void *, long, const void *, long, const havoc_mi355x_pair_job *, int, uint32_t *);
hipError_t launch_satd(hipStream_t, int S, int maxw, int maxh, const void *, long, const void *, long, const havoc_mi355x_pair_job *, int, int32_t *);
hipError_t launch_satd_multi(hipStream_t, int S, int maxw, int maxh, const void *, long, const void *, long, const havoc_mi355x_satd_multi_job *, int, int32_t *);
hipError_t launch_ssd_linear(hipStream_t, const uint8_t *, const uint8_t *, int, int32_t *);
hipError_t launch_pad_block(hipStream_t, int S, void *, long, int, int, long, int, int, int, int, int);
hipError_t launch_derive_bs(hipStream_t, const havoc_mi355x_cell *, long, int, int, int8_t *, uint8_t *);
hipError_t launch_deblock(hipStream_t, int S, int bd, void *, long, void *, void *, long, int, int, const int8_t *, const uint8_t *, int, int, int, int);
hipError_t launch_interp_planes(hipStream_t, int S, int bd, void *, long, const void *, long, int, int, int, int);
hipError_t launch_pred_uni(hipStream_t, int S, int taps, int bd, int maxw, int maxh, void *, long, const void *, long, const havoc_mi355x_pred_uni_job *, int);
hipError_t launch_pred_bi(hipStream_t, int S, int taps, int bd, int maxw, int maxh, void *, long, const void *, long, const havoc_mi355x_pred_bi_job *, int);
hipError_t launch_pred_uni_classes(hipStream_t, int S, int taps, int bd, void *, long, const void *, long, const havoc_mi355x_pred_uni_job *, const int count[4]);
hipError_t launch_pred_bi_classes(hipStream_t, int S, int taps, int bd, void *, long, const void *, long, const havoc_mi355x_pred_bi_job *, const int count[4]);
hipError_t launch_subtract_bi(hipStream_t, int S, int bd, void *, long, const void *, long, const void *, long, const havoc_mi355x_subtract_bi_job *, int);
hipError_t launch_subpel_satd(hipStream_t, int S, int taps, int bd, int maxw, int maxh, const void *, long, const void *, long, const havoc_mi355x_pred_uni_job *, int,
                              int32_t *);
hipError_t launch_intra(hipStream_t, int S, int log2, int bd, void *, long, const void *, const havoc_mi355x_intra_job *, int);
hipError_t launch_intra_satd35(hipStream_t, int S, int log2, int bd, const void *, long, const void *, const havoc_mi355x_intra_search_job *, int, int32_t *);
hipError_t launch_transform(hipStream_t, int bd, int log2, int tr, int16_t *, const int16_t *, long, const havoc_mi355x_tu_job *, int);
hipError_t launch_inverse_transform(hipStream_t, int mode, int bd, int log2, int tr, void *, long, const void *, long, int16_t *, const int16_t *,
                                    const havoc_mi355x_tu_job *, int);
hipError_t launch_level_stats(hipStream_t, const int16_t *, const int32_t *, int, int32_t *);
hipError_t launch_quantize(hipStream_t, int16_t *, const int16_t *, const havoc_mi355x_quant_job *, int, int32_t *);
hipError_t launch_quantize_inverse(hipStream_t, int16_t *, const int16_t *, const havoc_mi355x_quant_job *, int);
hipError_t launch_quantize_reconstruct(hipStream_t, int log2, uint8_t *, long, const uint8_t *, long, const int16_t *, const havoc_mi355x_tu_job *, int);
hipError_t launch_residual(hipStream_t, int S, int16_t *, long, const int32_t *, const void *, long, const void *, long, const havoc_mi355x_pair_job *, int);
hipError_t launch_tu_forward(hipStream_t, int S, int bd, int log2, int tr, int16_t *, const void *, long, const void *, long, const havoc_mi355x_tu_fused_job *, int);
hipError_t launch_tu_forward_scan(hipStream_t, int S, int bd, int log2, int16_t *, const void *, long, const void *, long, const havoc_mi355x_tu_fused_job *, int,
                                  const havoc_mi355x_rdoq_job *, int16_t *, void *);
hipError_t launch_intra_measure(hipStream_t, int S, int bd, int log2, int16_t *, int16_t *, int32_t *, void *, uint32_t *, const void *, long, const void *, long,
                                const havoc_mi355x_tu_fused_job *, int, int);
hipError_t launch_tu_reconstruct(hipStream_t, int S, int bd, int log2, int tr, int scale, int shift, void *, long, const void *, long, const void *, long, const int16_t *,
                                 const havoc_mi355x_tu_fused_job *, int, uint32_t *);
size_t rdoq_workspace_bytes(int njobs);
hipError_t launch_rdoq(hipStream_t, int bd, int log2, int16_t *, const int16_t *, const uint8_t *, const havoc_mi355x_rdoq_job *, int, int32_t *, void *);
hipError_t launch_rdoq_prescanned(hipStream_t, int bd, int log2, int16_t *, const int16_t *, const uint8_t *, const havoc_mi355x_rdoq_job *, int, int32_t *, void *);
hipError_t launch_residual_rate(hipStream_t, int log2, const int16_t *, const uint8_t *, const havoc_mi355x_residual_rate_job *, int, int64_t *, uint8_t *);
hipError_t launch_intra_rate(hipStream_t, int log2, const int16_t *, const uint8_t *, const uint8_t *, const havoc_mi355x_intra_rate_job *, int, int64_t *, uint8_t *, uint8_t *);
hipError_t launch_tree_rate(hipStream_t, int log2Cb, int depth, const int16_t *, const int16_t *, const uint8_t *, const uint8_t *, const havoc_mi355x_tree_rate_job *, int, int64_t *,
                            uint32_t *, uint8_t *, uint8_t *);
hipError_t launch_pu_rate(hipStream_t, const uint8_t *, const havoc_mi355x_pu_rate_job *, int, const havoc_mi355x_pu_slice *, int64_t *, uint8_t *);
hipError_t launch_pu_decide(hipStream_t, const int32_t *, const int32_t *, int, const int64_t *, const int32_t *, const int32_t *, const int32_t *, int32_t, const uint8_t *,
                            int64_t *, int32_t *, int64_t *, uint8_t *);
hipError_t launch_cu_close(hipStream_t, const uint8_t *, const uint8_t *, const uint8_t *, const int64_t *, const havoc_mi355x_rqt_choice *, const havoc_mi355x_rqt_tree_choice *,
                           const int64_t *, const int32_t *, const havoc_mi355x_cu_close_job *, int, int, int32_t, havoc_mi355x_cu_choice *, uint8_t *, uint8_t *);
hipError_t launch_unit_pred_ssd(hipStream_t, int S, const void *, long, const void *, long, const void *, long, const void *, long, const havoc_mi355x_pred_ssd_job *, int,
                                int32_t *);
hipError_t launch_unit_pred_select(hipStream_t, int S, const void *, const void *, void *, long, void *, long, const int32_t *, const int32_t *, const int64_t *,
                                   const havoc_mi355x_pred_select_job *, int, int64_t *, int32_t *);
size_t cqt_decide_workspace_bytes(int nctus);
hipError_t launch_cqt_decide(hipStream_t, int width, int height, int ctbLog2, int minCbLog2, int flags, const uint8_t *, const int32_t *, const havoc_mi355x_cu_choice *, int,
                             void *work, havoc_mi355x_cqt_ctu *, havoc_mi355x_cqt_node *, int8_t *, uint8_t *);
hipError_t launch_cqt_commit(hipStream_t, const havoc_mi355x_cqt_commit_args &);
hipError_t launch_cqt_block_cells(hipStream_t, int width, int height, int minCbLog2, int qp, int dpb0, int dpb1, const havoc_mi355x_cqt_cell *, havoc_mi355x_cell *,
                                  long stride);
hipError_t launch_cqt_motion_store(hipStream_t, int width, int height, int minCbLog2, int refPoc0, int refPoc1, const havoc_mi355x_cqt_cell *, havoc_mi355x_col_cell *);
hipError_t launch_temporal_candidates(hipStream_t, const havoc_mi355x_temporal_params &, const havoc_mi355x_col_cell *, long stride, const void *pus, int n,
                                      havoc_mi355x_temporal_cand *);
hipError_t launch_intra_order(hipStream_t, const int32_t *, const havoc_mi355x_intra_mpm *, int, int32_t, int32_t *, int32_t *, int32_t *, int32_t *);
hipError_t launch_intra_expand(hipStream_t, const havoc_mi355x_intra_search_job *, const int32_t *, const int32_t *, const int32_t *, const int32_t *, int, int, int, int, int,
                               int, int, int, havoc_mi355x_intra_job *, havoc_mi355x_tu_fused_job *, havoc_mi355x_rdoq_job *, int32_t *, int32_t *);
hipError_t launch_intra_decide(hipStream_t, const havoc_mi355x_intra_mpm *, const int32_t *, const int32_t *, const int32_t *, const int32_t *, const uint32_t *,
                               const int32_t *, const havoc_mi355x_tu_fused_job *, int, int, int32_t, havoc_mi355x_intra_choice *, havoc_mi355x_tu_fused_job *,
                               const int64_t *rates);
hipError_t launch_intra_rate_jobs(hipStream_t, const havoc_mi355x_intra_mpm *, const int32_t *, const int32_t *, const int32_t *, const havoc_mi355x_rdoq_job *, int, int,
                                  havoc_mi355x_intra_rate_job *);
hipError_t launch_intra_fill_spare(hipStream_t, const int32_t *, int, int, havoc_mi355x_intra_job *, havoc_mi355x_tu_fused_job *, havoc_mi355x_rdoq_job *, int32_t *, int32_t *);
hipError_t launch_intra_gather(hipStream_t, int S, const havoc_mi355x_intra_chain_layout *, const void *, const int32_t *, const uint8_t *,
                               const havoc_mi355x_intra_chain_part *, int, const havoc_mi355x_intra_search_job *, void *, havoc_mi355x_intra_mpm *);
hipError_t launch_intra_commit(hipStream_t, int S, const havoc_mi355x_intra_chain_layout *, void *, uint8_t *, const havoc_mi355x_intra_chain_part *, int, const void *,
                               const int32_t *, int);
hipError_t launch_rqt_decide(hipStream_t, const havoc_mi355x_rqt_unit *, int, const int32_t *, const int32_t *, const havoc_mi355x_rqt_size sizes[4], long, int, int, int32_t,
                             havoc_mi355x_rqt_choice *, const int64_t *const *rates);
hipError_t launch_rqt_decide_tree(hipStream_t, const havoc_mi355x_rqt_unit *, int, const int32_t *, const int32_t *, const havoc_mi355x_rqt_size sizes[4],
                                  const havoc_mi355x_rqt_size csizes[4], const havoc_mi355x_rqt_chroma_at *, const int64_t *, const uint32_t *, long, int, int, long, long, int, int,
                                  int32_t, havoc_mi355x_rqt_choice *, havoc_mi355x_rqt_tree_choice *);
hipError_t launch_rqt_decide_units(hipStream_t, const havoc_mi355x_rqt_unit *, int, const int32_t *, const int32_t *, const havoc_mi355x_rqt_size sizes[4],
                                   const havoc_mi355x_rqt_size csizes[4], const havoc_mi355x_rqt_chroma_at *, const int64_t *, const uint32_t *, int32_t,
                                   havoc_mi355x_rqt_choice *, havoc_mi355x_rqt_tree_choice *);
hipError_t launch_block_cells(hipStream_t, int, int, int, int, const int16_t *, const havoc_mi355x_rqt_unit *, const havoc_mi355x_rqt_choice *, int, havoc_mi355x_cell *, bool);
hipError_t launch_merge_decide(hipStream_t, const int32_t *, const int32_t *, const int32_t *, int, int64_t, int64_t *, int32_t *);
hipError_t launch_merge_jobs(hipStream_t, const havoc_mi355x_field_layout *, const int16_t *, const int32_t *, const int32_t *, int, int, havoc_mi355x_pred_bi_job *,
                             havoc_mi355x_pred_bi_job *, havoc_mi355x_pred_bi_job *, int16_t *);
hipError_t launch_pred_jobs(hipStream_t, const havoc_mi355x_field_layout *, const int16_t *, int, const int32_t *, const int32_t *, int, int, int, const int32_t *,
                            havoc_mi355x_pred_uni_job *);
size_t search_workspace_bytes(int width, int height);
hipError_t launch_search_list(hipStream_t, int S, const havoc_mi355x_search_params *, const void *, long, long, const void *, long, long, const void *, long, long, const void *,
                              int, void *);
hipError_t launch_search_bi_list(hipStream_t, int S, const havoc_mi355x_search_params *, const void *, long, long, const void *, long, long, const void *, long, long, const void *,
                                 long, const void *, const int16_t *, int, void *);
hipError_t launch_search_picture_uni(hipStream_t, int S, const havoc_mi355x_search_params *, const int64_t *, const void *, long, long, const void *, const long *, long,
                                     const void *, long, const long *, const void *, const int32_t *, int, int, int, void *, void *, int16_t *, void *, int, const int32_t *);
hipError_t launch_search_wait_rows(hipStream_t, const void *, int, int, int, int *);
hipError_t launch_sao_stats(hipStream_t, int S, int bd, const void *, long, const void *, long, const havoc_mi355x_sao_stats_job *, int, int64_t *);
hipError_t launch_sao_band_chroma(hipStream_t, int S, int bd, const void *, long, const void *, long, const havoc_mi355x_sao_chroma_job *, int, int64_t *);
hipError_t launch_sao_filter(hipStream_t, int S, int bd, void *, long, const void *, long, const havoc_mi355x_sao_job *, int);
// ... 11 lines not shown
```

turingcodec_amd/havoc.py:

```python
import ctypes as C
import os

import numpy as np

_HERE = os.path.dirname(os.path.abspath(__file__))
LIB_PATH = os.environ.get("HAVOC_MI355X_LIB") or os.path.join(_HERE, "libhavoc_mi355x.so")

_vp = C.c_void_p
_ip = C.c_ssize_t
_i = C.c_int



def search_workspace(width, height):
    L, _ = _load()
    return int(L.havoc_mi355x_search_workspace(width, height))


class HavocError(RuntimeError):
    pass


def _load():
    if not os.path.exists(LIB_PATH):
        raise HavocError(f"{LIB_PATH} is missing: build it with `python -c 'import __graft_entry__ as g; g.build()'` "
                         "(make -C turingcodec_amd/csrc).  There is no fallback path.")
    L = C.CDLL(LIB_PATH)
    L.havoc_mi355x_last_error.restype = C.c_char_p
    L.havoc_mi355x_version.restype = C.c_char_p
    sig = {
        "create": [C.POINTER(_vp), _i, _vp],
        "destroy": [_vp],
        "set_stream": [_vp, _vp],
        "sync": [_vp],
        "sync_spin": [_vp],
        "device_info": [_vp, C.POINTER(C.c_int64)],
        "malloc": [_vp, C.POINTER(_vp), C.c_size_t],
        "free": [_vp, _vp],
        "h2d": [_vp, _vp, _vp, C.c_size_t],
        "d2h": [_vp, _vp, _vp, C.c_size_t],
        "host_alloc": [_vp, C.c_size_t, C.POINTER(_vp), C.POINTER(_vp)],
        "host_free": [_vp, _vp],
        "h2d_async": [_vp, _vp, _vp, C.c_size_t],
        "d2h_async": [_vp, _vp, _vp, C.c_size_t],
        "copy_2d": [_vp, _vp, C.c_size_t, _vp, C.c_size_t, C.c_size_t, C.c_size_t, _i],
        "picture_create": [_vp, _i, _i, _i, _i, _i, _i, C.POINTER(_vp)],
        "picture_destroy": [_vp, _vp],
        "picture_plane": [_vp, _i, C.POINTER(_vp), C.POINTER(C.c_int64), C.POINTER(_ip), C.POINTER(_i), C.POINTER(_i), C.POINTER(_i)],
        "picture_upload_yuv": [_vp, _vp, _vp, _i, _i, _i],
        "picture_upload_plane": [_vp, _vp, _i, _vp, _ip, _i],
        "picture_download_plane": [_vp, _vp, _i, _vp, _ip, _i],
        "picture_pad": [_vp, _vp],
        "picture_phase_planes": [_vp, _vp, C.POINTER(_vp), C.POINTER(_ip), C.POINTER(C.c_int64)],
        "timer_start": [_vp],
        "timer_stop_ms": [_vp, C.POINTER(C.c_float)],
        "graph_begin": [_vp],
        "graph_end": [_vp, C.POINTER(_vp)],
        "graph_launch": [_vp, _vp],
        "graph_destroy": [_vp],
        "fork": [_vp, _i],
        "lane": [_vp, _i],
        "join": [_vp],
        "sad": [_vp, _i, _vp, _ip, _vp, _ip, _vp, _i, _vp],
        "sad4": [_vp, _i, _vp, _ip, _vp, _ip, _vp, _i, _vp],
        "sad4_runs": [_vp, _i, _vp, _ip, _vp, _ip, _vp, _i, _vp, _i, _vp],
        "sad4_make_runs": [_vp, _i, _i, _ip, _i, _vp],
        "pad_block": [_vp, _i, _vp, C.c_int64, _i, _i, _ip, _i, _i, _i, _i, _i],
        "sad_surface": [_vp, _i, _i, _i, _i, _vp, _ip, _vp, _ip, _vp, _i, _vp],
        "deblock": [_vp, _i, _i, _vp, _ip, _vp, _vp, _ip, _i, _i, _vp, _vp, _i, _i, _i, _i],
        "derive_bs": [_vp, _vp, _ip, _i, _i, _vp, _vp],
        "ssd": [_vp, _i, _vp, _ip, _vp, _ip, _vp, _i, _vp],
        "satd": [_vp, _i, _i, _i, _vp, _ip, _vp, _ip, _vp, _i, _vp],
        "satd_multi": [_vp, _i, _i, _i, _vp, _ip, _vp, _ip, _vp, _i, _vp],
        "ssd_linear": [_vp, _vp, _vp, _i, _vp],
        "pred_uni": [_vp, _i, _i, _i, _i, _i, _vp, _ip, _vp, _ip, _vp, _i],
        "pred_bi": [_vp, _i, _i, _i, _i, _i, _vp, _ip, _vp, _ip, _vp, _i],
        "subtract_bi": [_vp, _i, _i, _vp, _ip, _vp, _ip, _vp, _ip, _vp, _i],
        "pred_uni_classes": [_vp, _i, _i, _i, _vp, _ip, _vp, _ip, _vp, C.POINTER(C.c_int32)],
        "pred_bi_classes": [_vp, _i, _i, _i, _vp, _ip, _vp, _ip, _vp, C.POINTER(C.c_int32)],
        "intra": [_vp, _i, _i, _i, _vp, _ip, _vp, _vp, _i],
        "intra_satd35": [_vp, _i, _i, _i, _vp, _ip, _vp, _vp, _i, _vp],
        "subpel_satd": [_vp, _i, _i, _i, _i, _i, _vp, _ip, _vp, _ip, _vp, _i, _vp],
        "interp_planes": [_vp, _i, _i, _vp, _ip, _vp, _ip, _i, _i, _i, _i],
        "residual": [_vp, _i, _vp, _ip, _vp, _vp, _ip, _vp, _ip, _vp, _i],
        "transform": [_vp, _i, _i, _i, _vp, _vp, _ip, _vp, _i],
        "inverse_transform": [_vp, _i, _i, _i, _vp, _vp, _vp, _i],
        "inverse_transform_add": [_vp, _i, _i, _i, _i, _vp, _ip, _vp, _ip, _vp, _vp, _i],
        "tu_forward": [_vp, _i, _i, _i, _i, _vp, _vp, _ip, _vp, _ip, _vp, _i],
        "tu_reconstruct": [_vp, _i, _i, _i, _i, _i, _i, _vp, _ip, _vp, _ip, _vp, _ip, _vp, _vp, _i, _vp],
        "intra_measure": [_vp, _i, _i, _i, _vp, _vp, _vp, _vp, _vp, _vp, _ip, _vp, _ip, _vp, _i, _i],
        "level_stats": [_vp, _vp, _vp, _i, _vp],
        "search_motion_uni": [_vp, _i, _vp, _vp, C.c_int64, _ip, _vp, C.c_int64, _ip, _vp, _ip, C.c_int64, _vp, _i, _vp],
        "rqt_decide": [_vp, _vp, _i, _vp, _vp, _vp, C.c_int64, C.c_ssize_t, _i, _i, _vp],
        "block_cells": [_vp, _i, _i, _i, _i, _vp, _vp, _vp, _i, _vp],
        "intra_gather": [_vp, _i, _vp, _vp, _vp, _vp, _vp, _i, _vp, _vp, _vp],
        "intra_commit": [_vp, _i, _vp, _vp, _vp, _vp, _i, _vp, _vp, _i],
        "intra_fill_spare": [_vp, _vp, _i, _i, _vp, _vp, _vp, _vp, _vp],
        "merge_jobs": [_vp, _vp, _vp, _vp, _vp, _i, _i, _vp, _vp, _vp, _vp],
        "merge_decide": [_vp, _vp, _vp, _vp, _i, C.c_int64, _vp, _vp],
        "pred_jobs": [_vp, _vp, _vp, _i, _vp, _vp, _i, _i, _i, _vp, _vp],
        "search_motion_bi": [_vp, _i, _vp, _vp, C.c_int64, _ip, _vp, C.c_int64, _ip, _vp, _ip, C.c_int64, _vp, C.c_int64, _vp, _vp, _i, _vp],
        "search_picture_uni": [_vp, _i, _vp, _vp, _vp, C.c_int64, _ip, _vp, _vp, _ip, _vp, _ip, _vp, _vp, _vp, _i, _i, _i, _vp, _vp, _vp, _vp, _i],
        "search_gate": [_vp, _vp],
        "search_wait_rows": [_vp, _vp, _i, _i, _i, _vp],
        "block_cells_add": [_vp, _i, _i, _i, _i, _vp, _vp, _vp, _i, _vp],
        "intra_order": [_vp, _vp, _vp, _i, C.c_int32, _vp, _vp, _vp, _vp],
        "intra_expand": [_vp, _vp, _vp, _vp, _vp, _vp, _i, _i, _i, _i, _i, _i, _i, _i, _vp, _vp, _vp, _vp, _vp],
        "intra_decide": [_vp, _vp, _vp, _vp, _vp, _vp, _vp, _vp, _vp, _i, _i, C.c_int32, _vp, _vp],
        "quantize": [_vp, _vp, _vp, _vp, _i, _vp],
        "quantize_inverse": [_vp, _vp, _vp, _vp, _i],
        "quantize_reconstruct": [_vp, _i, _vp, _ip, _vp, _ip, _vp, _vp, _i],
        "rdoq": [_vp, _i, _i, _vp, _vp, _vp, _vp, _i, _vp, _vp, C.c_size_t],
        "tu_forward_scan": [_vp, _i, _i, _i, _vp, _vp, _ip, _vp, _ip, _vp, _i, _vp, _vp, _vp, C.c_size_t],
        "rdoq_prescanned": [_vp, _i, _i, _vp, _vp, _vp, _vp, _i, _vp, _vp, C.c_size_t],
        "residual_rate": [_vp, _i, _vp, _vp, _vp, _i, _vp, _vp],
        "intra_rate": [_vp, _i, _vp, _vp, _vp, _vp, _i, _vp, _vp, _vp],
        "intra_rate_jobs": [_vp, _vp, _vp, _vp, _vp, _vp, _i, _i, _vp],
        "tree_rate": [_vp, _i, _i, _vp, _vp, _vp, _vp, _vp, _i, _vp, _vp, _vp, _vp],
        "pu_rate": [_vp, _vp, _vp, _i, _vp, _vp, _vp],
        "pu_decide": [_vp, _vp, _vp, _i, _vp, _vp, _vp, _vp, C.c_int32, _vp, _vp, _vp, _vp, _vp],
        "cu_close": [_vp, _vp, _vp, _vp, _vp, _vp, _vp, _vp, _vp, _vp, _i, _i, C.c_int32, _vp, _vp, _vp],
        "unit_pred_ssd": [_vp, _i, _vp, C.c_ssize_t, _vp, C.c_ssize_t, _vp, C.c_ssize_t, _vp, C.c_ssize_t, _vp, _i, _vp],
        "unit_pred_select": [_vp, _i, _vp, _vp, _vp, C.c_ssize_t, _vp, C.c_ssize_t, _vp, _vp, _vp, _vp, _i, _vp, _vp],
        "cqt_decide": [_vp, _i, _i, _i, _i, _i, _vp, _vp, _vp, _i, _vp, C.c_size_t, _vp, _vp, _vp, _vp],
        "cqt_commit": [_vp, _vp],
        "cqt_block_cells": [_vp, _i, _i, _i, _i, _i, _i, _vp, _vp, _ip],
        "cqt_motion_store": [_vp, _i, _i, _i, _i, _i, _i, _vp, _vp],
        "temporal_candidates": [_vp, _vp, _vp, _ip, _vp, _i, _vp],
        "intra_decide_rated": [_vp, _vp, _vp, _vp, _vp, _vp, _vp, _vp, _vp, _vp, _i, _i, C.c_int32, _vp, _vp],
        "rqt_decide_rated": [_vp, _vp, _i, _vp, _vp, _vp, _vp, C.c_int64, C.c_ssize_t, _i, _i, _vp],
        "rqt_decide_tree": [_vp, _vp, _i, _vp, _vp, _vp, _vp, _vp, _vp, _vp, C.c_int64, C.c_ssize_t, _i, C.c_int64, C.c_int64, C.c_ssize_t, _i, _i, _vp, _vp],
        "rqt_decide_units": [_vp, _vp, _i, _vp, _vp, _vp, _vp, _vp, _vp, _vp, _i, _vp, _vp],
        "sao_stats": [_vp, _i, _i, _vp, _ip, _vp, _ip, _vp, _i, _vp],
        "sao_filter": [_vp, _i, _i, _vp, _ip, _vp, _ip, _vp, _i],
        "sao_band_chroma": [_vp, _i, _i, _vp, _ip, _vp, _ip, _vp, _i, _vp],
        "sao_estimate": [_vp, _i, _i, C.c_int32, _i, _vp, _vp, _ip, _ip, _vp, _vp, _ip, _ip, _vp, _vp, _ip, _ip, _vp, _i, _vp, C.c_size_t, _vp],
        "sao_decide": [_vp, _i, _i, C.c_int32, _i, _vp, _vp, _ip, _ip, _vp, _vp, _ip, _ip, _vp, _vp, _ip, _ip, _vp, _i, _i, _vp, _i, _i, _vp, C.c_size_t,
                       _vp],
        "sao_apply": [_vp, _i, _i, _i, _i, _i, _i, _vp, _vp, _vp, _ip, _ip, _vp, _vp, _vp, _ip, _ip, _vp, _vp, _vp, _ip],
    }
    L.havoc_mi355x_rdoq_lambda.argtypes = [C.c_double, _i, C.POINTER(C.c_int32), C.POINTER(C.c_int32)]
    L.havoc_mi355x_rdoq_lambda.restype = None
    L.havoc_mi355x_rdoq_workspace.argtypes = [_i]
    L.havoc_mi355x_rdoq_workspace.restype = C.c_size_t
    L.havoc_mi355x_sao_workspace.argtypes = [_i]
    L.havoc_mi355x_sao_workspace.restype = C.c_size_t
    L.havoc_mi355x_sao_decide_workspace.argtypes = [_i]
    L.havoc_mi355x_sao_decide_workspace.restype = C.c_size_t
    L.havoc_mi355x_cqt_decide_workspace.argtypes = [_i]
    L.havoc_mi355x_cqt_decide_workspace.restype = C.c_size_t
    L.havoc_mi355x_search_workspace.argtypes = [_i, _i]
    L.havoc_mi355x_search_workspace.restype = C.c_size_t
    for name, args in sig.items():
        f = getattr(L, "havoc_mi355x_" + name)
        f.argtypes = args
        f.restype = None if name in ("destroy", "graph_destroy", "picture_destroy") else _i
    return L, sorted(sig)


def exported_symbols():
    _, names = _load()
    return ["havoc_mi355x_" + n for n in names] + ["havoc_mi355x_last_error", "havoc_mi355x_version", "havoc_mi355x_rdoq_lambda", "havoc_mi355x_rdoq_workspace",
# ... 366 lines not shown
        L, _ = _load()
        jobs = np.ascontiguousarray(jobs, np.int32)
        runs = np.zeros((max(1, len(jobs)), 8), np.int32)
        n = L.havoc_mi355x_sad4_make_runs(jobs.ctypes.data, len(jobs), max_run, stride if stride is not None else 0, S, runs.ctypes.data)
        if n < 0:
            raise HavocError("havoc_mi355x_sad4_make_runs failed")
        return np.ascontiguousarray(runs[:n])

    def ssd_d(self, a, sa, b, sb, jobs, out):
        self._ck(self.L.havoc_mi355x_ssd(self.h, self._S(a), _ptr(a), sa, _ptr(b), sb, _ptr(jobs), jobs.shape[0], _ptr(out)))

    def satd_d(self, a, sa, b, sb, jobs, out, max_w=64, max_h=64):
        self._ck(self.L.havoc_mi355x_satd(self.h, self._S(a), max_w, max_h, _ptr(a), sa, _ptr(b), sb, _ptr(jobs), jobs.shape[0], _ptr(out)))

    def satd_multi_d(self, a, sa, b, sb, jobs, out, max_w=64, max_h=64):
        self._ck(self.L.havoc_mi355x_satd_multi(self.h, self._S(a), max_w, max_h, _ptr(a), sa, _ptr(b), sb, _ptr(jobs), jobs.shape[0], _ptr(out)))

    def pred_uni_d(self, taps, bd, dst, sd, ref, sr, jobs, max_w=64, max_h=64):
        self._ck(self.L.havoc_mi355x_pred_uni(self.h, self._S(ref), taps, bd, max_w, max_h, _ptr(dst), sd, _ptr(ref), sr, _ptr(jobs), jobs.shape[0]))

    def pred_bi_d(self, taps, bd, dst, sd, ref, sr, jobs, max_w=64, max_h=64):
        self._ck(self.L.havoc_mi355x_pred_bi(self.h, self._S(ref), taps, bd, max_w, max_h, _ptr(dst), sd, _ptr(ref), sr, _ptr(jobs), jobs.shape[0]))

    @staticmethod
    def field_layout(pic_width, pic_height, luma_stride, luma_pad, luma_plane_elems, chroma_stride, chroma_pad, chroma_plane_elems, search_range=64):
        return (C.c_int32 * 12)(pic_width, pic_height, search_range, (pic_width + 3) // 4, luma_stride, luma_pad, luma_plane_elems, chroma_stride, chroma_pad, chroma_plane_elems, 0, 0)

    def rqt_decide_d(self, units, zero_at, one_at, sizes, rec_origin, rec_stride, dump_off, rl_q16, out):
        self._ck(self.L.havoc_mi355x_rqt_decide(self.h, _ptr(units), units.shape[0], _ptr(zero_at), _ptr(one_at), sizes.ctypes.data, int(rec_origin), int(rec_stride), int(dump_off),
                                                int(rl_q16), _ptr(out)))

    def rqt_decide_rated_d(self, units, zero_at, one_at, sizes, rates, rec_origin, rec_stride, dump_off, rl_q16, out):
        self._ck(self.L.havoc_mi355x_rqt_decide_rated(self.h, _ptr(units), units.shape[0], _ptr(zero_at), _ptr(one_at), sizes.ctypes.data, rates.ctypes.data, int(rec_origin),
                                                      int(rec_stride), int(dump_off), int(rl_q16), _ptr(out)))

    def rqt_decide_tree_d(self, units, zero_at, one_at, sizes, csizes, chroma_at, tree_rates, tree_cbf, rec_origin, rec_stride, dump_off, cb_origin, cr_origin, c_stride,
                          c_dump_off, rl_q16, out, tree_out):
        self._ck(self.L.havoc_mi355x_rqt_decide_tree(self.h, _ptr(units), units.shape[0], _ptr(zero_at), _ptr(one_at), sizes.ctypes.data, csizes.ctypes.data, _ptr(chroma_at),
                                                     _ptr(tree_rates), _ptr(tree_cbf), int(rec_origin), int(rec_stride), int(dump_off), int(cb_origin), int(cr_origin),
                                                     int(c_stride), int(c_dump_off), int(rl_q16), _ptr(out), _ptr(tree_out)))

    def rqt_decide_units_d(self, units, zero_at, one_at, sizes, csizes, chroma_at, tree_rates, tree_cbf, rl_q16, out, tree_out):
        self._ck(self.L.havoc_mi355x_rqt_decide_units(self.h, _ptr(units), units.shape[0], _ptr(zero_at), _ptr(one_at), sizes.ctypes.data, csizes.ctypes.data, _ptr(chroma_at),
                                                      _ptr(tree_rates), _ptr(tree_cbf), int(rl_q16), _ptr(out), _ptr(tree_out)))

    def block_cells_add_d(self, width, height, qp, dpb_index0, field, units, decisions, cells):
        self._ck(self.L.havoc_mi355x_block_cells_add(self.h, width, height, qp, dpb_index0, _ptr(field), _ptr(units), _ptr(decisions), units.shape[0], _ptr(cells)))

    def block_cells_d(self, width, height, qp, dpb_index0, field, units, decisions, cells):
        self._ck(self.L.havoc_mi355x_block_cells(self.h, width, height, qp, dpb_index0, _ptr(field), _ptr(units), _ptr(decisions), units.shape[0], _ptr(cells)))

    @staticmethod
    def intra_chain_layout(pic_width, pic_height, stride, pad, cells_per_row, bit_depth, ctb_log2=6, strong_intra_smoothing=1):
        return (C.c_int32 * 8)(pic_width, pic_height, stride, pad, cells_per_row, bit_depth, ctb_log2, int(bool(strong_intra_smoothing)))

    def intra_gather_a(self, S, layout, rec, owner, modes, parts, n, jobs, neighbours, mpm):
        self._ck(self.L.havoc_mi355x_intra_gather(self.h, S, layout, rec, owner, modes, parts, n, jobs, neighbours, mpm))

    def intra_commit_a(self, S, layout, rec, modes, parts, n, blocks, mode, mode_stride=1):
        self._ck(self.L.havoc_mi355x_intra_commit(self.h, S, layout, rec, modes, parts, n, blocks, mode, mode_stride))

    def merge_jobs_d(self, layout, field, x0, y0, log2, luma_jobs, cb_jobs, cr_jobs, vectors):
        self._ck(self.L.havoc_mi355x_merge_jobs(self.h, layout, _ptr(field), _ptr(x0), _ptr(y0), x0.shape[0], log2, _ptr(luma_jobs), _ptr(cb_jobs), _ptr(cr_jobs), _ptr(vectors)))

    def merge_decide_d(self, satd_y, satd_cb, satd_cr, n, lam_q16, cost, best):
        self._ck(self.L.havoc_mi355x_merge_decide(self.h, _ptr(satd_y), _ptr(satd_cb), _ptr(satd_cr), n, int(lam_q16), _ptr(cost), _ptr(best)))

    def pred_jobs_d(self, layout, field, lst, x0, y0, log2, plane, dst_off, jobs):
        self._ck(self.L.havoc_mi355x_pred_jobs(self.h, layout, _ptr(field), lst, _ptr(x0), _ptr(y0), x0.shape[0], log2, plane, _ptr(dst_off), _ptr(jobs)))

    @staticmethod
    def sort_by_class(jobs, w, h):
        big = np.maximum(np.asarray(w), np.asarray(h))
        cls = np.searchsorted([8, 16, 32], big, side="left")
        order = np.argsort(cls, kind="stable")
        counts = np.bincount(cls, minlength=4).astype(np.int32)
        return np.ascontiguousarray(np.asarray(jobs)[order]), counts, order

    def pred_classes_d(self, bi, taps, bd, dst, sd, ref, sr, jobs, counts):
        c = (C.c_int32 * 4)(*[int(v) for v in counts])
        f = self.L.havoc_mi355x_pred_bi_classes if bi else self.L.havoc_mi355x_pred_uni_classes
        self._ck(f(self.h, self._S(ref), taps, bd, _ptr(dst), sd, _ptr(ref), sr, _ptr(jobs), c))

    @staticmethod
    def size_classes(w, h):
        big = np.maximum(np.asarray(w), np.asarray(h))
        out = []
        for lo, hi in ((0, 8), (8, 16), (16, 32), (32, 64)):
            idx = np.flatnonzero((big > lo) & (big <= hi))
            if len(idx):
                out.append((idx, hi, hi))
        return out

    def subtract_bi_d(self, bd, dst, sd, pred, sp, src, ss, jobs):
        self._ck(self.L.havoc_mi355x_subtract_bi(self.h, self._S(src), bd, _ptr(dst), sd, _ptr(pred), sp, _ptr(src), ss, _ptr(jobs), jobs.shape[0]))

    def intra_d(self, bd, log2, dst, sd, nb, jobs):
        self._ck(self.L.havoc_mi355x_intra(self.h, self._S(nb), bd, log2, _ptr(dst), sd, _ptr(nb), _ptr(jobs), jobs.shape[0]))

    def search_gate(self, rows_ready=None):
        self._gate = rows_ready
        self._ck(self.L.havoc_mi355x_search_gate(self.h, _ptr(rows_ready) if rows_ready is not None else None))

    def search_wait_rows(self, work, width, height, ctu_row, gave_up):
        self._ck(self.L.havoc_mi355x_search_wait_rows(self.h, _ptr(work), width, height, ctu_row, _ptr(gave_up)))

    def search_picture_uni_d(self, S, params, mvp_rate, src, src_origin, src_stride, ref, ref_origin, ref_stride, phase, plane_elems, phase_origin, pus, ctu_first, ctus_x, ctus_y,
                             n_pus, out, out_bi, field, work):
        ro, po, mr = (C.c_int64 * 2)(*[int(v) for v in ref_origin]), (C.c_int64 * 2)(*[int(v) for v in phase_origin]), (C.c_int64 * 2)(*[int(v) for v in mvp_rate])
        self._ck(self.L.havoc_mi355x_search_picture_uni(self.h, S, C.byref(params), mr, _ptr(src), int(src_origin), src_stride, _ptr(ref), ro, ref_stride, _ptr(phase), plane_elems, po,
                                                        _ptr(pus), _ptr(ctu_first), ctus_x, ctus_y, n_pus, _ptr(out), _ptr(out_bi) if out_bi is not None else None, _ptr(field),
                                                        _ptr(work), 0))

    def interp_planes_d(self, bd, planes, plane_elems, ref, stride, x0, y0, width, height):
        self._ck(self.L.havoc_mi355x_interp_planes(self.h, self._S(ref), bd, _ptr(planes), plane_elems, _ptr(ref), stride, x0, y0, width, height))

    def interp_planes(self, bd, ref, stride, x0, y0, width, height):
        planes = self.zeros(16 * len(ref), ref.dtype)
        self.interp_planes_d(bd, planes, len(ref), self.up(ref), stride, x0, y0, width, height)
        return self.down(planes, ref.dtype).reshape(16, -1)

    def subpel_satd_d(self, taps, bd, max_w, max_h, src, ss, ref, sr, jobs, cost):
        self._ck(self.L.havoc_mi355x_subpel_satd(self.h, self._S(ref), taps, bd, max_w, max_h, _ptr(src), ss, _ptr(ref), sr, _ptr(jobs),
                                                 jobs.shape[0], _ptr(cost)))

    def subpel_satd(self, taps, bd, src, ss, ref, sr, jobs):
        jobs = np.asarray(jobs, np.int32)
        out = np.zeros(len(jobs), np.int32)
        s, r = self.up(src), self.up(ref)
        big = np.maximum(jobs[:, 2], jobs[:, 3])
        for lo, hi in ((0, 8), (8, 16), (16, 32), (32, 64)):
            idx = np.flatnonzero((big > lo) & (big <= hi))
            if len(idx):
                cost = self.zeros(len(idx), np.int32)
                self.subpel_satd_d(taps, bd, hi, hi, s, ss, r, sr, self._jobs(jobs[idx], 8), cost)
                out[idx] = self.down(cost, np.int32)
        return out

    def intra_satd35_d(self, bd, log2, src, ss, nb, jobs, cost):
        self._ck(self.L.havoc_mi355x_intra_satd35(self.h, self._S(src), bd, log2, _ptr(src), ss, _ptr(nb), _ptr(jobs), jobs.shape[0], _ptr(cost)))

    def residual_d(self, res, sres, res_off, src, ss, pred, sp, jobs):
        self._ck(self.L.havoc_mi355x_residual(self.h, self._S(src), _ptr(res), sres, _ptr(res_off), _ptr(src), ss, _ptr(pred), sp, _ptr(jobs), jobs.shape[0]))

    def transform_d(self, bd, tr, log2, coeffs, res, sres, jobs):
        self._ck(self.L.havoc_mi355x_transform(self.h, bd, tr, log2, _ptr(coeffs), _ptr(res), sres, _ptr(jobs), jobs.shape[0]))

    def inverse_transform_d(self, bd, tr, log2, res, coeffs, jobs):
        self._ck(self.L.havoc_mi355x_inverse_transform(self.h, bd, tr, log2, _ptr(res), _ptr(coeffs), _ptr(jobs), jobs.shape[0]))

    def inverse_transform_add_d(self, bd, tr, log2, dst, sd, pred, sp, coeffs, jobs):
        self._ck(self.L.havoc_mi355x_inverse_transform_add(self.h, self._S(pred), bd, tr, log2, _ptr(dst), sd, _ptr(pred), sp, _ptr(coeffs), _ptr(jobs), jobs.shape[0]))

    def tu_forward_d(self, bd, tr, log2, coeffs, src, ss, pred, sp, jobs):
        self._ck(self.L.havoc_mi355x_tu_forward(self.h, self._S(src), bd, tr, log2, _ptr(coeffs), _ptr(src), ss, _ptr(pred), sp, _ptr(jobs), jobs.shape[0]))

    def tu_reconstruct_d(self, bd, tr, log2, scale, shift, rec, sr, pred, sp, src, ss, levels, jobs, ssd):
        self._ck(self.L.havoc_mi355x_tu_reconstruct(self.h, self._S(src), bd, tr, log2, scale, shift, _ptr(rec), sr, _ptr(pred), sp, _ptr(src), ss,
                                                    _ptr(levels), _ptr(jobs), jobs.shape[0], _ptr(ssd)))

    def intra_measure_d(self, bd, log2, coeffs, coeffs_dct, satd, rec0, ssd0, src, ss, pred, sp, jobs, with_satd=True):
        self._ck(self.L.havoc_mi355x_intra_measure(self.h, self._S(src), bd, log2, _ptr(coeffs), _ptr(coeffs_dct) if coeffs_dct is not None else None,
                                                   _ptr(satd) if satd is not None else None, _ptr(rec0), _ptr(ssd0), _ptr(src), ss, _ptr(pred), sp, _ptr(jobs),
                                                   jobs.shape[0], 1 if with_satd else 0))

    def level_stats_d(self, levels, jobs, njobs, out):
# ... 562 lines not shown
```

turingcodec_amd/step.py:

```python
import numpy as np


class DeviceFrame:

    def __init__(self, hv, wl, use_planes=True, fused_tu=True, ime_range=None, skip=(), rdoq=True, pred_launches="merged", scan_in_forward=True, sad4_runs=True):
        import torch
        self.sad4_runs = sad4_runs
        from turingcodec_amd import havoc as _havoc
        self.rdoq = bool(rdoq) and wl.mix == "ra"
        self.skip = set(skip)
        self.hv, self.wl, self.use_planes, self.fused_tu, self.ime_range = hv, wl, use_planes, fused_tu, ime_range
        self.pred_launches, self.scan_in_forward = pred_launches, scan_in_forward
        up = hv.up
        dt = wl.dtype
        S = wl.S
        store = np.concatenate([wl.luma, np.zeros(wl.plane_len, dt)])
        self.luma = up(store)
        self.chroma = up(np.concatenate([wl.chroma, np.zeros(2 * wl.cplane_len, dt)]))
        z = lambda n, d: hv.zeros(n, d)
        self.pred = z(wl.pred_len, dt)
        self.cpred = z(wl.cpred_len, dt)
        self.bi = z(wl.bi_len + 4096, dt)
        self.cbi = z(len(wl.bi4) * 1024 + 1024, dt)
        self.sbi = z(len(wl.subtract_bi) * 4096, dt)
        self.j_sad4, self.j_sad = up(wl.sad4), up(wl.sad)
        self.j_runs = up(hv.sad4_make_runs(wl.sad4, 0, wl.stride, wl.S)) if sad4_runs and len(wl.sad4) else None
        self.o_sad4, self.o_sad = z(4 * len(wl.sad4), np.int32), z(len(wl.sad), np.int32)
        if ime_range is not None:
            side = 2 * ime_range + 1
            sj = np.zeros((len(wl.me_search), 8), np.int32)
            sj[:, :4] = wl.me_search
            sj[:, 4] = np.arange(len(sj)) * side * side
            self.j_surf, self.o_surf = up(sj), z(len(sj) * side * side, np.int32)
        self.j_sbi = up(wl.subtract_bi)
        self.j_satd = up(wl.satd_inter)
        self.o_satd = z(len(wl.satd_inter), np.int32)
        self.subpel = {hi: dict(jobs=up(j), cost=z(len(j), np.int32)) for hi, j in wl.subpel.items() if len(j)}
        if self.use_planes:
            pl = wl.plane_len
            self.planes = z(32 * pl, dt)
            self.planes[0:pl].copy_(self.luma[pl:2 * pl])
            self.planes[16 * pl:17 * pl].copy_(self.luma[2 * pl:3 * pl])
            self.subpel_planes = {c: dict(jobs=up(j), cost=z(16 * len(j), np.int32)) for c, j in wl.subpel_planes.items() if len(j)}
        self.intra = {}
        for log2, j in wl.intra.items():
            if len(j):
                self.intra[log2] = dict(jobs=up(j), nb=up(wl.intra_nb[log2]), dst=z(len(j) << (2 * log2), dt))
        self.isearch = {}
        for log2, j in wl.intra_search.items():
            if len(j):
                self.isearch[log2] = dict(jobs=up(j), nb=up(wl.intra_search_nb[log2]), cost=z(35 * len(j), np.int32))
        self.tu = {}
        bd = wl.bit_depth
        qp = wl.qp
        from turingcodec_amd.workload import quant_params, dequant_params
        for (log2, tr), g in wl.tu.items():
            m = len(g["jobs"])
            if not m:
                continue
            nn = g["n"]
            qscale, qshift, qoffset = quant_params(qp, log2, bd, wl.mix == "ai")
            dscale, dshift = dequant_params(qp, log2, bd)
            qj = np.zeros((m, 8), np.int32)
            qj[:, 0] = qj[:, 1] = g["jobs"][:, 0]
            qj[:, 2] = nn * nn
            qj[:, 3], qj[:, 4], qj[:, 5] = qscale, qshift, qoffset
            dj = qj.copy()
            dj[:, 3], dj[:, 4] = dscale, dshift
            self.tu[(log2, tr)] = dict(jobs=up(g["jobs"]), src=up(g["src"]), res_off=up(g["res_off"]), n=nn,
                                       res=z(m * nn * nn, np.int16), coef=z(m * nn * nn, np.int16),
                                       level=z(m * nn * nn, np.int16), deq=z(m * nn * nn, np.int16),
                                       qjobs=up(qj), djobs=up(dj), cbf=z(m, np.int32), rec=z(m * nn * nn, dt),
                                       jssd=up(g["ssd"]), ossd=z(len(g["ssd"]), np.uint32), dscale=dscale, dshift=dshift)
            fj = g["jobs"].copy()
            fj[:, 1] = g["src"][:, 0]
            extra = g["ssd"][m:]
            self.tu[(log2, tr)].update(fjobs=up(fj), jssd_x=up(extra) if len(extra) else None, ossd_x=z(max(1, len(extra)), np.uint32))
            if self.rdoq:
                rj = wl.rdoq_jobs((log2, tr), _havoc.rdoq_lambda(wl.rdoq_lambda, dscale))
                self.tu[(log2, tr)]["rjobs"] = torch.from_numpy(rj.view(np.uint8).reshape(-1)).to(hv.device)
                self.tu[(log2, tr)]["rwork"] = hv.rdoq_workspace(len(rj))
        self.rdoq_states = torch.from_numpy(np.ascontiguousarray(wl.rdoq_states).reshape(-1)).to(hv.device)
        self.recon = {}
        for comp, tabs in wl.recon.items():
            for log2, g in tabs.items():
                dscale, dshift = dequant_params(qp, log2, bd)
                self.recon[(comp, log2)] = dict(jobs=up(g["jobs"]), levels=up(g["levels"]), ssd=z(len(g["jobs"]), np.uint32), n=g["n"],
                                                dscale=dscale, dshift=dshift)
        self.dbk_data = torch.from_numpy(np.ascontiguousarray(wl.deblock_blocks[0])).to(hv.device)
        self.dbk_bs = torch.from_numpy(np.ascontiguousarray(wl.deblock_blocks[1])).to(hv.device)
        self.init_refs = (self.luma[wl.plane_len:3 * wl.plane_len].clone(), self.chroma[wl.cplane_len:3 * wl.cplane_len].clone())
        self.launches = self._make_launches()
        torch.cuda.synchronize()
        if not self.rdoq:
            for name, fn in self.launches:
                if name.startswith(("residual", "transform", "tu_forward")):
                    fn()
            for g in self.tu.values():
                hv.quantize_d(g["level"], g["coef"], g["qjobs"], g["cbf"])
        hv.sync()

    def _make_launches(self):
        hv, wl = self.hv, self.wl
        bd, st, cst = wl.bit_depth, wl.stride, wl.cstride
        L = []
        chains = []

        def chain(*items):
            items = [it for it in items if it[0] not in self.skip]
            if items:
                chains.append(list(range(len(L), len(L) + len(items))))
                L.extend(items)

        inter = wl.mix == "ra"
        if not inter:
            pass
        elif self.ime_range is None:
            if self.j_runs is not None:
                chain(("sad4", lambda: hv.sad4_runs_d(self.luma, st, self.luma, st, self.j_sad4, self.j_runs, self.o_sad4)))
            else:
                chain(("sad4", lambda: hv.sad4_d(self.luma, st, self.luma, st, self.j_sad4, self.o_sad4)))
        else:
            chain(("sad_surface", lambda: hv.sad_surface_d(self.luma, st, self.luma, st, self.ime_range, 64, 64, self.j_surf, self.o_surf)))
        if inter:
            chain(("sad", lambda: hv.sad_d(self.luma, st, self.luma, st, self.j_sad, self.o_sad)))
        if not inter:
            pass
        elif self.use_planes:
            pl, m = wl.plane_len, wl.plane_margin
            x0, y0, rw, rh = 96 - m, 96 - m, wl.width + 2 * m, wl.height + 2 * m
            items = [("interp_planes", lambda r=r: hv.interp_planes_d(bd, self.planes[16 * r * pl:], pl, self.luma[(1 + r) * pl:], st, x0, y0, rw, rh))
                     for r in (0, 1)]
            for (mw, mh), g in sorted(self.subpel_planes.items(), reverse=True):
                items.append(("satd_planes", lambda g=g, mw=mw, mh=mh: hv.satd_multi_d(self.luma, st, self.planes, st, g["jobs"], g["cost"], mw, mh)))
            chain(*items)
        else:
            for hi, g in sorted(self.subpel.items(), reverse=True):
                chain(("subpel_satd", lambda g=g, hi=hi: hv.subpel_satd_d(8, bd, hi, hi, self.luma, st, self.luma, st, g["jobs"], g["cost"])))
        def classes(name, jobs, wcol, fn):
            jobs_np = np.asarray(jobs)
            return [(name, lambda j=hv.up(np.ascontiguousarray(jobs_np[idx])), mw=mw, mh=mh: fn(j, mw, mh))
                    for idx, mw, mh in hv.size_classes(jobs_np[:, wcol], jobs_np[:, wcol + 1])]

        if inter and self.pred_launches == "merged":
            def merged(name, jobs, wcol, bi, taps, dst, sd, ref, sr):
                srt, counts, _ = hv.sort_by_class(np.asarray(jobs), np.asarray(jobs)[:, wcol], np.asarray(jobs)[:, wcol + 1])
                return (name, lambda j=hv.up(srt), c=counts: hv.pred_classes_d(bi, taps, bd, dst, sd, ref, sr, j, c))
            chain(merged("pred_uni8", wl.uni8, 2, False, 8, self.pred, 64, self.luma, st),
                  ("satd_inter", lambda: hv.satd_d(self.luma, st, self.pred, 64, self.j_satd, self.o_satd)))
            chain(merged("pred_uni4", wl.uni4, 2, False, 4, self.cpred, 32, self.chroma, cst))
            chain(merged("pred_bi8", wl.bi8, 3, True, 8, self.bi, 64, self.luma, st),
                  ("subtract_bi", lambda: hv.subtract_bi_d(bd, self.sbi, 64, self.bi, 64, self.luma, st, self.j_sbi)),
                  merged("pred_bi4", wl.bi4, 3, True, 4, self.cbi, 32, self.chroma, cst))
        elif inter:
            chain(*classes("pred_uni8", wl.uni8, 2, lambda j, mw, mh: hv.pred_uni_d(8, bd, self.pred, 64, self.luma, st, j, mw, mh)),
                  ("satd_inter", lambda: hv.satd_d(self.luma, st, self.pred, 64, self.j_satd, self.o_satd)))
            chain(*classes("pred_uni4", wl.uni4, 2, lambda j, mw, mh: hv.pred_uni_d(4, bd, self.cpred, 32, self.chroma, cst, j, mw, mh)))
            chain(*classes("pred_bi8", wl.bi8, 3, lambda j, mw, mh: hv.pred_bi_d(8, bd, self.bi, 64, self.luma, st, j, mw, mh)),
                  ("subtract_bi", lambda: hv.subtract_bi_d(bd, self.sbi, 64, self.bi, 64, self.luma, st, self.j_sbi)),
                  *classes("pred_bi4", wl.bi4, 3, lambda j, mw, mh: hv.pred_bi_d(4, bd, self.cbi, 32, self.chroma, cst, j, mw, mh)))
        for log2, g in sorted(self.isearch.items(), reverse=True):
            chain(("intra_satd35", lambda g=g, log2=log2: hv.intra_satd35_d(bd, log2, self.luma, st, g["nb"], g["jobs"], g["cost"])))
        for log2, g in sorted(self.intra.items(), reverse=True):
            n = 1 << log2
            chain(("intra", lambda g=g, log2=log2, n=n: hv.intra_d(bd, log2, g["dst"], n, g["nb"], g["jobs"])))
        for (log2, tr), g in sorted(self.tu.items(), reverse=True):
            n = g["n"]
            rdq = ("rdoq", lambda g=g, log2=log2: hv.rdoq_d(bd, log2, g["level"], g["coef"], self.rdoq_states, g["rjobs"], g["cbf"], g["rwork"]))
            if self.fused_tu:
                fwd = ("tu_forward", lambda g=g, log2=log2, tr=tr: hv.tu_forward_d(bd, tr, log2, g["coef"], self.luma, st, self.luma, st, g["fjobs"]))
                items = [("tu_reconstruct", lambda g=g, log2=log2, tr=tr, n=n: hv.tu_reconstruct_d(
                    bd, tr, log2, g["dscale"], g["dshift"], g["rec"], n, self.luma, st, self.luma, st, g["level"], g["fjobs"], g["ossd"]))]
                if g["jssd_x"] is not None:
                    items.append(("ssd", lambda g=g, n=n: hv.ssd_d(self.luma, st, g["rec"], n, g["jssd_x"], g["ossd_x"])))
                if self.rdoq and self.scan_in_forward and log2 >= 4 and tr == 0:
                    chain(("tu_forward", lambda g=g, log2=log2: hv.tu_forward_scan_d(bd, log2, g["coef"], self.luma, st, self.luma, st, g["fjobs"], g["rjobs"],
                                                                                      g["level"], g["rwork"])),
                          ("rdoq", lambda g=g, log2=log2: hv.rdoq_prescanned_d(bd, log2, g["level"], g["coef"], self.rdoq_states, g["rjobs"], g["cbf"], g["rwork"])),
                          *items)
                elif self.rdoq:
                    chain(fwd, rdq, *items)
                elif inter:
                    chain(fwd)
                    chain(*items)
                else:
                    chain(fwd, ("quantize", lambda g=g: hv.quantize_d(g["level"], g["coef"], g["qjobs"], g["cbf"])), *items)
                continue
            front = [("residual", lambda g=g, n=n: hv.residual_d(g["res"], n, g["res_off"], self.luma, st, self.luma, st, g["src"])),
                     ("transform", lambda g=g, n=n, log2=log2, tr=tr: hv.transform_d(bd, tr, log2, g["coef"], g["res"], n, g["jobs"]))]
            back = [("quantize_inverse", lambda g=g: hv.quantize_inverse_d(g["deq"], g["level"], g["djobs"])),
                    ("inverse_transform_add", lambda g=g, log2=log2, tr=tr, n=n: hv.inverse_transform_add_d(
                        bd, tr, log2, g["rec"], n, self.luma, st, g["deq"], g["jobs"])),
                    ("ssd", lambda g=g, n=n: hv.ssd_d(self.luma, st, g["rec"], n, g["jssd"], g["ossd"]))]
            if self.rdoq:
                chain(*front, rdq, *back)
            else:
                chain(*front)
                chain(*back)
        if inter and "recon" not in self.skip:
            items = []
            for (comp, log2), g in sorted(self.recon.items(), key=lambda kv: (-kv[0][1], kv[0][0])):
                plane, stv = (self.luma, st) if comp == "y" else (self.chroma, cst)
                items.append(("recon", lambda g=g, log2=log2, plane=plane, stv=stv: hv.tu_reconstruct_d(
                    bd, 0, log2, g["dscale"], g["dshift"], plane, stv, plane, stv, plane, stv, g["levels"], g["jobs"], g["ssd"])))
            pl_, cpl_ = wl.plane_len, wl.cplane_len
            if "deblock" not in self.skip:
                items.append(("deblock", lambda: hv.deblock_d(bd, self.luma, 3 * pl_ + 96 * st + 96, st, self.chroma, 3 * cpl_ + 48 * cst + 48,
                                                               4 * cpl_ + 48 * cst + 48, cst, wl.width, wl.height, self.dbk_data, self.dbk_bs)))
            chain(*items)
        self.chains = chains
        return L

    def step(self, nlanes=1):
        if nlanes <= 1:
            for _, fn in self.launches:
                fn()
            return
        hv = self.hv
        assign = getattr(self, "assign", None) or [list(range(k, len(self.chains), nlanes)) for k in range(nlanes)]
        hv.fork(nlanes)
        for k, lane in enumerate(assign):
            hv.lane(k)
            for ci in lane:
                for idx in self.chains[ci]:
                    self.launches[idx][1]()
        hv.join()

    def chain_times_ms(self):
        hv, out = self.hv, []
        for ch in self.chains:
            run = lambda: [self.launches[i][1]() for i in ch]
            run()
            hv.timer_start()
            for _ in range(3):
                run()
            out.append(hv.timer_stop_ms() / 3)
# ... 200 lines not shown
```

Baseline: 1574 frames/s.

## Fuse SATD into uni prediction and SubtractBi into bi prediction kernels

Adds fused launch paths that compute the inter SATD cost directly from the in-register uni-predicted rows, and write the SubtractBi residual from the in-register bi-predicted rows. The host matches follower jobs to prediction jobs by destination offset and size, packing the source and destination offsets into spare job fields. This removes two separate launches per frame and the re-read of the prediction buffer from memory. In exchange the prediction kernel gains register pressure and extra loads, and the satd path needs a cross-lane reduction. It falls back to the old path when jobs do not match one to one.

```diff
diff --git a/include/havoc_mi355x.h b/include/havoc_mi355x.h
--- a/include/havoc_mi355x.h
+++ b/include/havoc_mi355x.h
@@ -198,6 +198,12 @@
                                   intptr_t stride_ref, const havoc_mi355x_pred_uni_job *d_jobs, const int32_t count[4]);
 int havoc_mi355x_pred_bi_classes(havoc_mi355x_ctx *ctx, int S, int taps, int bitDepth, void *d_dst, intptr_t stride_dst, const void *d_ref,
                                  intptr_t stride_ref, const havoc_mi355x_pred_bi_job *d_jobs, const int32_t count[4]);
+int havoc_mi355x_pred_uni_satd_classes(havoc_mi355x_ctx *ctx, int S, int taps, int bitDepth, void *d_dst, intptr_t stride_dst, const void *d_ref,
+                                       intptr_t stride_ref, const havoc_mi355x_pred_uni_job *d_jobs, const int32_t count[4], const void *d_src,
+                                       intptr_t stride_src, int32_t *d_cost);
+int havoc_mi355x_pred_bi_subtract_classes(havoc_mi355x_ctx *ctx, int S, int taps, int bitDepth, void *d_dst, intptr_t stride_dst, const void *d_ref,
+                                          intptr_t stride_ref, const havoc_mi355x_pred_bi_job *d_jobs, const int32_t count[4], const void *d_src,
+                                          intptr_t stride_src, void *d_sub, intptr_t stride_sub);
 int havoc_mi355x_subtract_bi(havoc_mi355x_ctx *ctx, int S, int bitDepth, void *d_dst, intptr_t stride_dst,
                              const void *d_pred, intptr_t stride_pred, const void *d_src, intptr_t stride_src,
                              const havoc_mi355x_subtract_bi_job *d_jobs, int njobs);
diff --git a/turingcodec_amd/csrc/api.hip b/turingcodec_amd/csrc/api.hip
--- a/turingcodec_amd/csrc/api.hip
+++ b/turingcodec_amd/csrc/api.hip
@@ -502,6 +502,25 @@
     return check(launch_pred_bi_classes(LS(ctx), S, taps, bitDepth, d_dst, stride_dst, d_ref, stride_ref, d_jobs, count), "pred_bi_classes");
 }
 
+int havoc_mi355x_pred_uni_satd_classes(havoc_mi355x_ctx *ctx, int S, int taps, int bitDepth, void *d_dst, intptr_t stride_dst, const void *d_ref, intptr_t stride_ref,
+                                       const havoc_mi355x_pred_uni_job *d_jobs, const int32_t count[4], const void *d_src, intptr_t stride_src, int32_t *d_cost)
+{
+    REQUIRE_CTX(); REQUIRE_S(); REQUIRE_BD(); REQUIRE(taps == 8 || taps == 4, "taps must be 8 or 4"); REQUIRE(count != nullptr, "null count");
+    REQUIRE(d_src != nullptr && d_cost != nullptr, "null source / cost");
+    return check(launch_pred_uni_satd_classes(LS(ctx), S, taps, bitDepth, d_dst, stride_dst, d_ref, stride_ref, d_jobs, count, d_src, stride_src, d_cost),
+                 "pred_uni_satd_classes");
+}
+
+int havoc_mi355x_pred_bi_subtract_classes(havoc_mi355x_ctx *ctx, int S, int taps, int bitDepth, void *d_dst, intptr_t stride_dst, const void *d_ref, intptr_t stride_ref,
+                                          const havoc_mi355x_pred_bi_job *d_jobs, const int32_t count[4], const void *d_src, intptr_t stride_src, void *d_sub,
+                                          intptr_t stride_sub)
+{
+    REQUIRE_CTX(); REQUIRE_S(); REQUIRE_BD(); REQUIRE(taps == 8 || taps == 4, "taps must be 8 or 4"); REQUIRE(count != nullptr, "null count");
+    REQUIRE(d_src != nullptr && d_sub != nullptr, "null source / SubtractBi destination");
+    return check(launch_pred_bi_subtract_classes(LS(ctx), S, taps, bitDepth, d_dst, stride_dst, d_ref, stride_ref, d_jobs, count, d_src, stride_src, d_sub, stride_sub),
+                 "pred_bi_subtract_classes");
+}
+
 int havoc_mi355x_subtract_bi(havoc_mi355x_ctx *ctx, int S, int bitDepth, void *d_dst, intptr_t stride_dst, const void *d_pred, intptr_t stride_pred,
                              const void *d_src, intptr_t stride_src, const havoc_mi355x_subtract_bi_job *d_jobs, int njobs)
 {
diff --git a/turingcodec_amd/csrc/block_bodies.h b/turingcodec_amd/csrc/block_bodies.h
--- /dev/null
+++ b/turingcodec_amd/csrc/block_bodies.h
@@ -0,0 +1,189 @@
+#pragma once
+
+#include "common.h"
+
+namespace havoc_gpu {
+
+template <int S, int N>
+__device__ __forceinline__ void load_diff_row(const char *a, const char *b, int (&d)[N])
+{
+    if (S == 1)
+    {
+        if (N == 8)
+        {
+            const u32x2 va = ld8(a), vb = ld8(b);
+#pragma unroll
+            for (int x = 0; x < 4; ++x)
+            {
+                d[x] = (int)((va.x >> (8 * x)) & 0xff) - (int)((vb.x >> (8 * x)) & 0xff);
+                d[x + 4] = (int)((va.y >> (8 * x)) & 0xff) - (int)((vb.y >> (8 * x)) & 0xff);
+            }
+        }
+        else
+        {
+            const uint32_t va = ld4(a), vb = ld4(b);
+#pragma unroll
+            for (int x = 0; x < 4; ++x) d[x] = (int)((va >> (8 * x)) & 0xff) - (int)((vb >> (8 * x)) & 0xff);
+        }
+    }
+    else
+    {
+        if (N == 8)
+        {
+            const u32x4 va = ld16(a), vb = ld16(b);
+            const uint32_t wa[4] = {va.x, va.y, va.z, va.w}, wb[4] = {vb.x, vb.y, vb.z, vb.w};
+#pragma unroll
+            for (int x = 0; x < 4; ++x)
+            {
+                d[2 * x] = (int)(wa[x] & 0xffff) - (int)(wb[x] & 0xffff);
+                d[2 * x + 1] = (int)(wa[x] >> 16) - (int)(wb[x] >> 16);
+            }
+        }
+        else
+        {
+            const u32x2 va = ld8(a), vb = ld8(b);
+            d[0] = (int)(va.x & 0xffff) - (int)(vb.x & 0xffff);
+            d[1] = (int)(va.x >> 16) - (int)(vb.x >> 16);
+            d[2] = (int)(va.y & 0xffff) - (int)(vb.y & 0xffff);
+            d[3] = (int)(va.y >> 16) - (int)(vb.y >> 16);
+        }
+    }
+}
+
+template <int S, int G>
+__device__ __forceinline__ int satd_block_share(const char *a, long stride_a, const char *b, long stride_b, int w, int h, int l)
+{
+    typedef typename Sample<S>::T T;
+    const long sab = stride_a * S, sbb = stride_b * S;
+    int acc = 0;
+    if (((w | h) & 7) == 0)
+    {
+        const int tw = w >> 3;
+        const FastDiv fd(tw);
+        for (int it = l; it < tw * (h >> 3) * 8; it += G)
+        {
+            const int tile = it >> 3, r = it & 7;
+            const int ty = fd.div(tile), tx = tile - ty * tw;
+            const char *pa8 = a + (long)(ty * 8 + r) * sab + tx * 8 * S, *pb8 = b + (long)(ty * 8 + r) * sbb + tx * 8 * S;
+            if (S == 1)
+            {
+                const u32x2 va = ld8(pa8), vb = ld8(pb8);
+                const uint32_t m = 0x00ff00ffu;
+                uint32_t p[4] = {pk_sub(va.x & m, vb.x & m), pk_sub((va.x >> 8) & m, (vb.x >> 8) & m),
+                                 pk_sub(va.y & m, vb.y & m), pk_sub((va.y >> 8) & m, (vb.y >> 8) & m)};
+                acc += satd_rows_pk<8>(p, r);
+            }
+            else
+            {
+                int d[8];
+                load_diff_row<S, 8>(pa8, pb8, d);
+                acc += satd_rows<S, 8>(d, r);
+            }
+        }
+    }
+    else if (((w | h) & 3) == 0)
+    {
+        const int tw = w >> 2;
+        const FastDiv fd(tw);
+        for (int it = l; it < tw * (h >> 2) * 4; it += G)
+        {
+            const int tile = it >> 2, r = it & 3;
+            const int ty = fd.div(tile), tx = tile - ty * tw;
+            const char *pa4 = a + (long)(ty * 4 + r) * sab + tx * 4 * S, *pb4 = b + (long)(ty * 4 + r) * sbb + tx * 4 * S;
+            if (S == 1)
+            {
+                const uint32_t va = ld4(pa4), vb = ld4(pb4), m = 0x00ff00ffu;
+                uint32_t p[2] = {pk_sub(va & m, vb & m), pk_sub((va >> 8) & m, (vb >> 8) & m)};
+                acc += satd_rows_pk<4>(p, r);
+            }
+            else
+            {
+                int d[4];
+                load_diff_row<S, 4>(pa4, pb4, d);
+                acc += satd_rows<S, 4>(d, r);
+            }
+        }
+    }
+    else
+    {
+        const int tw = w >> 1;
+        const FastDiv fd(tw);
+        for (int t = l; t < tw * (h >> 1); t += G)
+        {
+            const int ty = fd.div(t), tx = t - ty * tw;
+            const T *p = reinterpret_cast<const T *>(a + (long)(2 * ty) * sab) + 2 * tx;
+            const T *q = reinterpret_cast<const T *>(b + (long)(2 * ty) * sbb) + 2 * tx;
+            const int d0 = (int)p[0] - (int)q[0], d1 = (int)p[1] - (int)q[1];
+            const int d2 = (int)p[stride_a] - (int)q[stride_b], d3 = (int)p[stride_a + 1] - (int)q[stride_b + 1];
+            int sum = abs(d0 + d1 + d2 + d3) + abs(d0 - d1 + d2 - d3) + abs(d0 + d1 - d2 - d3) + abs(d0 - d1 - d2 + d3);
+            if (S == 2) sum >>= 2;
+            acc += sum;
+        }
+    }
+    return acc;
+}
+
+template <int S>
+__device__ __forceinline__ void load_quad(const char *p, uint32_t (&v)[S])
+{
+    if constexpr (S == 1) v[0] = ld4(p);
+    else
+    {
+        const u32x2 t = ld8(p);
+        v[0] = t.x;
+        v[1] = t.y;
+    }
+}
+
+template <int S>
+__device__ __forceinline__ void subtract_bi_quad(char *dd, const uint32_t (&sv)[S], const uint32_t (&pv)[S], int maxv)
+{
+    const s16x2 zero = {0, 0}, top = {(short)maxv, (short)maxv};
+    auto sub_clip = [&](uint32_t a32, uint32_t b32) {
+        const s16x2 a = __builtin_bit_cast(s16x2, a32), b = __builtin_bit_cast(s16x2, b32);
+        return __builtin_bit_cast(uint32_t, __builtin_elementwise_min(__builtin_elementwise_max(a + a - b, zero), top));
+    };
+    if constexpr (S == 1)
+    {
+        const uint32_t lo = sub_clip(__builtin_amdgcn_perm(0u, sv[0], 0x0c010c00u), __builtin_amdgcn_perm(0u, pv[0], 0x0c010c00u));
+        const uint32_t hi = sub_clip(__builtin_amdgcn_perm(0u, sv[0], 0x0c030c02u), __builtin_amdgcn_perm(0u, pv[0], 0x0c030c02u));
+        st4(dd, __builtin_amdgcn_perm(hi, lo, 0x06040200u));
+    }
+    else
+        st8(dd, u32x2{sub_clip(sv[0], pv[0]), sub_clip(sv[1], pv[1])});
+}
+
+template <int S, int NL>
+__device__ __forceinline__ void subtract_bi_block(char *d, long stride_dst, const char *p, long stride_pred, const char *s, long stride_src, int w, int h, int maxv,
+                                                  int lane, int lean)
+{
+    typedef typename Sample<S>::T T;
+    if (lean && (w & 3) == 0 && w <= 4 * NL)
+    {
+        const int qpr = w >> 2;
+        const FastDiv fq(qpr);
+        const int y0 = fq.div(lane), q = lane - y0 * qpr, ystep = fq.div(NL);
+        if (y0 >= ystep) return;
+        const long db = stride_dst * S, pb = stride_pred * S, sb = stride_src * S;
+        char *dd = d + 4 * q * S + y0 * db;
+        const char *pp = p + 4 * q * S + y0 * pb, *ss = s + 4 * q * S + y0 * sb;
+        for (int y = y0; y < h; y += ystep, dd += ystep * db, pp += ystep * pb, ss += ystep * sb)
+        {
+            uint32_t sv[S], pv[S];
+            load_quad<S>(ss, sv);
+            load_quad<S>(pp, pv);
+            subtract_bi_quad<S>(dd, sv, pv, maxv);
+        }
+        return;
+    }
+    const FastDiv fd(w);
+    T *dt = reinterpret_cast<T *>(d);
+    const T *pt = reinterpret_cast<const T *>(p), *st = reinterpret_cast<const T *>(s);
+    for (int i = lane; i < w * h; i += NL)
+    {
+        const int y = fd.div(i), x = i - y * w;
+        dt[y * stride_dst + x] = (T)clip3(0, maxv, 2 * (int)st[y * stride_src + x] - (int)pt[y * stride_pred + x]);
+    }
+}
+
+}
diff --git a/turingcodec_amd/csrc/kernels_inter.hip b/turingcodec_amd/csrc/kernels_inter.hip
--- a/turingcodec_amd/csrc/kernels_inter.hip
+++ b/turingcodec_amd/csrc/kernels_inter.hip
@@ -3,8 +3,18 @@
 #include "common.h"
 #include "launch.h"
 #include "interp.h"
+#include "block_bodies.h"
 
 namespace havoc_gpu {
+
+struct PredFollow
+{
+    const char *src;
+    long stride_src;
+    int32_t *cost;
+    char *sub;
+    long stride_sub;
+};
 
 template <int MAXW, int MAXH, int G, bool BI>
 struct PredLds
@@ -139,9 +149,9 @@
 constexpr int kDppXor2 = 0x4E;
 
 template <int S>
-__device__ __forceinline__ void store_quad_rows(char *q, long dsb, const int (&v)[8], int c, int rowsLeft)
-{
-    if (S == 1)
+__device__ __forceinline__ void quad_rows(const int (&v)[8], int c, uint32_t (&row)[2][S])
+{
+    if constexpr (S == 1)
     {
         const uint32_t selA = (c & 1) ? 0x03070105u : 0x06020400u, selB = (c & 2) ? 0x03020706u : 0x05040100u;
 #pragma unroll
@@ -150,8 +160,7 @@
             const int *u = v + 4 * half;
             uint32_t d = (uint32_t)u[0] | ((uint32_t)u[1] << 8) | ((uint32_t)u[2] << 16) | ((uint32_t)u[3] << 24);
             d = __builtin_amdgcn_perm((uint32_t)dpp_mov<kDppXor1>((int)d), d, selA);
-            d = __builtin_amdgcn_perm((uint32_t)dpp_mov<kDppXor2>((int)d), d, selB);
-            if (c + 4 * half < rowsLeft) st4(q + 4 * half * dsb, d);
+            row[half][0] = __builtin_amdgcn_perm((uint32_t)dpp_mov<kDppXor2>((int)d), d, selB);
         }
     }
     else
@@ -166,8 +175,40 @@
             e0 = __builtin_amdgcn_perm((uint32_t)dpp_mov<kDppXor1>((int)e0), e0, selA);
             e1 = __builtin_amdgcn_perm((uint32_t)dpp_mov<kDppXor1>((int)e1), e1, selA);
             const uint32_t t = (uint32_t)dpp_mov<kDppXor2>((int)(hi ? e0 : e1));
-            if (c + 4 * half < rowsLeft) st8(q + 4 * half * dsb, u32x2{hi ? t : e0, hi ? e1 : t});
-        }
+            row[half][0] = hi ? t : e0;
+            row[half][1] = hi ? e1 : t;
+        }
+    }
+}
+
+template <int S>
+__device__ __forceinline__ void store_row(char *q, const uint32_t (&r)[S])
+{
+    if constexpr (S == 1) st4(q, r[0]);
+    else st8(q, u32x2{r[0], r[1]});
+}
+
+template <int S>
+__device__ __forceinline__ int quad_rows_satd(const uint32_t (&src)[2][S], const uint32_t (&row)[2][S], int r)
+{
+    if constexpr (S == 1)
+    {
+        const uint32_t s0 = src[0][0], s1 = src[1][0], m = 0x00ff00ffu;
+        uint32_t p[4] = {pk_sub(s0 & m, row[0][0] & m), pk_sub((s0 >> 8) & m, (row[0][0] >> 8) & m), pk_sub(s1 & m, row[1][0] & m),
+                         pk_sub((s1 >> 8) & m, (row[1][0] >> 8) & m)};
+        return satd_rows_pk<8>(p, r);
+    }
+    else
+    {
+        const uint32_t sv[4] = {src[0][0], src[0][1], src[1][0], src[1][1]}, pv[4] = {row[0][0], row[0][1], row[1][0], row[1][1]};
+        int d[8];
+#pragma unroll
+        for (int k = 0; k < 4; ++k)
+        {
+            d[2 * k] = (int)(sv[k] & 0xffff) - (int)(pv[k] & 0xffff);
+            d[2 * k + 1] = (int)(sv[k] >> 16) - (int)(pv[k] >> 16);
+        }
+        return satd_rows<S, 8>(d, r);
     }
 }
 
@@ -181,9 +222,24 @@
     return __ballot(w & 3) == 0;
 }
 
-template <int S, int TAPS, int MAXW, int MAXH, int G, bool BI>
+template <int JPW>
+__device__ __forceinline__ bool measured_in_tiles_of_eight(const int32_t *__restrict__ jobs, int njobs, int wg, int wgs)
+{
+    const int lane = threadIdx.x & (kWave - 1);
+    const int job = xcd_block(wg, wgs) * JPW + lane;
+    int odd = 0;
+    if (lane < JPW && job < njobs)
+    {
+        const int32_t *j = jobs + (long)job * 8;
+        odd = j[7] != 0 && ((j[2] | j[3]) & 7) != 0;
+    }
+    return __ballot(odd) == 0;
+}
+
+template <int S, int TAPS, int MAXW, int MAXH, int G, bool BI, bool FUSE = false>
 __device__ __forceinline__ void pred_workgroup_lean(char *lds, char *__restrict__ dst, long stride_dst, const char *__restrict__ ref, long stride_ref,
-                                                    const int32_t *__restrict__ jobs, int njobs, int bitDepth, int wg, int wgs)
+                                                    const int32_t *__restrict__ jobs, int njobs, int bitDepth, int wg, int wgs, const PredFollow *f = nullptr,
+                                                    bool inreg = false, int *share = nullptr)
 {
     typedef PredLeanLds<MAXW, MAXH, G, BI> L;
     constexpr int JPW = 256 / G;
@@ -281,10 +337,36 @@
     const FastDiv fw(w);
     char *d = dst + (long)j[0] * S;
     const int c = l & 3;
+    bool follow = false;
+    const char *fsrc = nullptr;
+    char *fsub = nullptr;
+    long ssb = 0, fsb = 0;
+    int sum = 0;
+    if constexpr (FUSE)
+    {
+        follow = inreg && (BI ? j[11] : j[7]) != 0;
+        fsrc = f->src + (long)j[BI ? 9 : 6] * S;
+        ssb = f->stride_src * S;
+        if constexpr (BI)
+        {
+            fsub = f->sub + (long)j[10] * S;
+            fsb = f->stride_sub * S;
+        }
+    }
     for (int it = l; it < w * groups; it += G)
     {
         const int gy = fw.div(it), x = it - gy * w;
         const int y0 = gy * 8;
+        uint32_t fsv[2][S] = {};
+        if constexpr (FUSE)
+        {
+            if (follow)
+            {
+#pragma unroll
+                for (int half = 0; half < 2; ++half)
+                    if (!BI || c + 4 * half < h - y0) load_quad<S>(fsrc + (y0 + c + 4 * half) * ssb + (x - c) * S, fsv[half]);
+            }
+        }
         int acc[8];
 #pragma unroll
         for (int r = 0; r < NREF; ++r)
@@ -328,8 +410,28 @@
             const int v = BI ? (acc[jj] + (1 << shift3)) >> (shift3 + 1) : (acc[jj] + (1 << (5 + shift3))) >> (6 + shift3);
             acc[jj] = clip3(0, maxv, v);
         }
-        store_quad_rows<S>(d + (y0 + c) * dsb + (x - c) * S, dsb, acc, c, h - y0);
-    }
+        uint32_t row[2][S];
+        quad_rows<S>(acc, c, row);
+        char *q = d + (y0 + c) * dsb + (x - c) * S;
+#pragma unroll
+        for (int half = 0; half < 2; ++half)
+            if (c + 4 * half < h - y0) store_row<S>(q + 4 * half * dsb, row[half]);
+        if constexpr (FUSE)
+        {
+            if (follow)
+            {
+                if constexpr (BI)
+                {
+#pragma unroll
+                    for (int half = 0; half < 2; ++half)
+                        if (c + 4 * half < h - y0) subtract_bi_quad<S>(fsub + (y0 + c + 4 * half) * fsb + (x - c) * S, fsv[half], row[half], maxv);
+                }
+                else
+                    sum += quad_rows_satd<S>(fsv, row, l & 7);
+            }
+        }
+    }
+    if constexpr (FUSE && !BI) *share = sum;
 }
 
 template <int S, int TAPS, int MAXW, int MAXH, int G, bool BI>
@@ -340,6 +442,62 @@
         pred_workgroup_lean<S, TAPS, MAXW, MAXH, G, BI>(lds, dst, stride_dst, ref, stride_ref, jobs, njobs, bitDepth, wg, wgs);
     else
         pred_workgroup_full<S, TAPS, MAXW, MAXH, G, BI>(lds, dst, stride_dst, ref, stride_ref, jobs, njobs, bitDepth, wg, wgs);
+}
+
+template <int G>
+__device__ __forceinline__ int job_sum(int v, int *s_red, int sub)
+{
+    if constexpr (G <= kWave) return group_sum<G>(v);
+    else
+    {
+        constexpr int W = G / kWave;
+        const int t = wave_sum(v);
+        if ((threadIdx.x & (kWave - 1)) == 0) s_red[threadIdx.x / kWave] = t;
+        __syncthreads();
+        int s = 0;
+#pragma unroll
+        for (int k = 0; k < W; ++k) s += s_red[sub * W + k];
+        return s;
+    }
+}
+
+template <int S, int TAPS, int MAXW, int MAXH, int G, bool BI>
+__device__ __forceinline__ void pred_workgroup_followed(char *lds, int *s_red, char *__restrict__ dst, long stride_dst, const char *__restrict__ ref, long stride_ref,
+                                                        const int32_t *__restrict__ jobs, int njobs, int bitDepth, int wg, int wgs, int lean, const PredFollow &f)
+{
+    constexpr int JPW = 256 / G;
+    const bool quads = lean && widths_are_quads<JPW, BI>(jobs, njobs, wg, wgs);
+    bool inreg = quads;
+    if constexpr (!BI) inreg = quads && measured_in_tiles_of_eight<JPW>(jobs, njobs, wg, wgs);
+    int share = 0;
+    if (quads)
+        pred_workgroup_lean<S, TAPS, MAXW, MAXH, G, BI, true>(lds, dst, stride_dst, ref, stride_ref, jobs, njobs, bitDepth, wg, wgs, &f, inreg, &share);
+    else
+        pred_workgroup_full<S, TAPS, MAXW, MAXH, G, BI>(lds, dst, stride_dst, ref, stride_ref, jobs, njobs, bitDepth, wg, wgs);
+
+    const int sub = threadIdx.x / G, l = threadIdx.x - sub * G;
+    const int job = xcd_block(wg, wgs) * JPW + sub;
+    const bool live = job < njobs;
+    const int32_t *j = jobs + (long)(live ? job : 0) * (BI ? 12 : 8);
+    const bool asked = live && (BI ? j[11] : j[7]) != 0;
+    if (!inreg)
+    {
+        __syncthreads();
+        const char *p = dst + (long)j[0] * S;
+        if constexpr (BI)
+        {
+            if (asked)
+                subtract_bi_block<S, G>(f.sub + (long)j[10] * S, f.stride_sub, p, stride_dst, f.src + (long)j[9] * S, f.stride_src, j[3], j[4], (1 << bitDepth) - 1, l,
+                                        lean);
+        }
+        else
+            share = satd_block_share<S, G>(f.src + (long)j[6] * S, f.stride_src, p, stride_dst, j[2], asked ? j[3] : 0, l);
+    }
+    if constexpr (!BI)
+    {
+        const int t = job_sum<G>(share, s_red, sub);
+        if (asked && l == 0) f.cost[j[7] - 1] = t;
+    }
 }
 
 template <int S, int TAPS, int MAXW, int MAXH, int G, bool BI>
@@ -372,58 +530,62 @@
                                                  bitDepth, wg - pc.firstWg[3], pc.firstWg[4] - pc.firstWg[3], lean);
 }
 
+template <int S, int TAPS, bool BI>
+__global__ __launch_bounds__(256) void k_pred_classes_fused(char *__restrict__ dst, long stride_dst, const char *__restrict__ ref, long stride_ref,
+                                                            const int32_t *__restrict__ jobs, PredClasses pc, int bitDepth, int lean, PredFollow f)
+{
+    __shared__ __attribute__((aligned(16))) char lds[PredLds<64, 64, 256, BI>::bytes];
+    __shared__ int s_red[256 / kWave];
+    constexpr int words = BI ? 12 : 8;
+    const int wg = blockIdx.x;
+    if (wg < pc.firstWg[1])
+        pred_workgroup_followed<S, TAPS, 8, 8, 8, BI>(lds, s_red, dst, stride_dst, ref, stride_ref, jobs, pc.count[0], bitDepth, wg, pc.firstWg[1], lean, f);
+    else if (wg < pc.firstWg[2])
+        pred_workgroup_followed<S, TAPS, 16, 16, 32, BI>(lds, s_red, dst, stride_dst, ref, stride_ref, jobs + (long)pc.count[0] * words, pc.count[1], bitDepth,
+                                                         wg - pc.firstWg[1], pc.firstWg[2] - pc.firstWg[1], lean, f);
+    else if (wg < pc.firstWg[3])
+        pred_workgroup_followed<S, TAPS, 32, 32, 128, BI>(lds, s_red, dst, stride_dst, ref, stride_ref, jobs + (long)(pc.count[0] + pc.count[1]) * words, pc.count[2],
+                                                          bitDepth, wg - pc.firstWg[2], pc.firstWg[3] - pc.firstWg[2], lean, f);
+    else
+        pred_workgroup_followed<S, TAPS, 64, 64, 256, BI>(lds, s_red, dst, stride_dst, ref, stride_ref, jobs + (long)(pc.count[0] + pc.count[1] + pc.count[2]) * words,
+                                                          pc.count[3], bitDepth, wg - pc.firstWg[3], pc.firstWg[4] - pc.firstWg[3], lean, f);
+}
+
+template <int S>
+__global__ __launch_bounds__(256) void k_pred_follow_satd(const char *__restrict__ src, long stride_src, const char *__restrict__ pred, long stride_pred,
+                                                          const int32_t *__restrict__ jobs, int njobs, int32_t *__restrict__ cost)
+{
+    const int job = xcd_block(blockIdx.x, gridDim.x) * 4 + __builtin_amdgcn_readfirstlane((int)threadIdx.x >> 6);
+    const int lane = threadIdx.x & 63;
+    const int32_t *j = jobs + (long)(job < njobs ? job : 0) * 8;
+    const bool asked = job < njobs && j[7] != 0;
+    const int t = wave_sum(satd_block_share<S, kWave>(src + (long)j[6] * S, stride_src, pred + (long)j[0] * S, stride_pred, j[2], asked ? j[3] : 0, lane));
+    if (asked && lane == 0) cost[j[7] - 1] = t;
+}
+
+template <int S>
+__global__ __launch_bounds__(256) void k_pred_follow_subtract(char *__restrict__ sub, long stride_sub, const char *__restrict__ pred, long stride_pred,
+                                                              const char *__restrict__ src, long stride_src, const int32_t *__restrict__ jobs, int njobs,
+                                                              int bitDepth, int lean)
+{
+    const int job = xcd_block(blockIdx.x, gridDim.x) * 4 + __builtin_amdgcn_readfirstlane((int)threadIdx.x >> 6);
+    if (job >= njobs) return;
+    const int32_t *j = jobs + (long)job * 12;
+    if (j[11] == 0) return;
+    subtract_bi_block<S, kWave>(sub + (long)j[10] * S, stride_sub, pred + (long)j[0] * S, stride_pred, src + (long)j[9] * S, stride_src, j[3], j[4],
+                                (1 << bitDepth) - 1, threadIdx.x & 63, lean);
+}
+
 template <int S>
 __global__ __launch_bounds__(256) void k_subtract_bi(char *__restrict__ dst, long stride_dst, const char *__restrict__ pred, long stride_pred,
                                                      const char *__restrict__ src, long stride_src, const int32_t *__restrict__ jobs, int njobs,
                                                      int bitDepth, int lean)
 {
-    typedef typename Sample<S>::T T;
     const int job = xcd_block(blockIdx.x, gridDim.x) * 4 + __builtin_amdgcn_readfirstlane((int)threadIdx.x >> 6);
-    const int lane = threadIdx.x & 63;
     if (job >= njobs) return;
     const int32_t *j = jobs + job * 8;
-    const int w = j[3], h = j[4];
-    T *d = reinterpret_cast<T *>(dst) + j[0];
-    const T *p = reinterpret_cast<const T *>(pred) + j[1];
-    const T *s = reinterpret_cast<const T *>(src) + j[2];
-    const int maxv = (1 << bitDepth) - 1;
-    if (lean && (w & 3) == 0 && w <= 4 * kWave)
-    {
-        const int qpr = w >> 2;
-        const FastDiv fq(qpr);
-        const int y0 = fq.div(lane), q = lane - y0 * qpr, ystep = fq.div(kWave);
-        if (y0 >= ystep) return;
-        const long db = stride_dst * S, pb = stride_pred * S, sb = stride_src * S;
-        char *dd = reinterpret_cast<char *>(d + 4 * q) + y0 * db;
-        const char *pp = reinterpret_cast<const char *>(p + 4 * q) + y0 * pb, *ss = reinterpret_cast<const char *>(s + 4 * q) + y0 * sb;
-        const s16x2 zero = {0, 0}, top = {(short)maxv, (short)maxv};
-        auto sub_clip = [&](uint32_t sv, uint32_t pv) {
-            const s16x2 a = __builtin_bit_cast(s16x2, sv), b = __builtin_bit_cast(s16x2, pv);
-            return __builtin_bit_cast(uint32_t, __builtin_elementwise_min(__builtin_elementwise_max(a + a - b, zero), top));
-        };
-        for (int y = y0; y < h; y += ystep, dd += ystep * db, pp += ystep * pb, ss += ystep * sb)
-        {
-            if (S == 1)
-            {
-                const uint32_t sv = ld4(ss), pv = ld4(pp);
-                const uint32_t lo = sub_clip(__builtin_amdgcn_perm(0u, sv, 0x0c010c00u), __builtin_amdgcn_perm(0u, pv, 0x0c010c00u));
-                const uint32_t hi = sub_clip(__builtin_amdgcn_perm(0u, sv, 0x0c030c02u), __builtin_amdgcn_perm(0u, pv, 0x0c030c02u));
-                st4(dd, __builtin_amdgcn_perm(hi, lo, 0x06040200u));
-            }
-            else
-            {
-                const u32x2 sv = ld8(ss), pv = ld8(pp);
-                st8(dd, u32x2{sub_clip(sv.x, pv.x), sub_clip(sv.y, pv.y)});
-            }
-        }
-        return;
-    }
-    const FastDiv fd(w);
-    for (int i = lane; i < w * h; i += kWave)
-    {
-        const int y = fd.div(i), x = i - y * w;
-        d[y * stride_dst + x] = (T)clip3(0, maxv, 2 * (int)s[y * stride_src + x] - (int)p[y * stride_pred + x]);
-    }
+    subtract_bi_block<S, kWave>(dst + (long)j[0] * S, stride_dst, pred + (long)j[1] * S, stride_pred, src + (long)j[2] * S, stride_src, j[3], j[4], (1 << bitDepth) - 1,
+                                threadIdx.x & 63, lean);
 }
 
 static int pred_lean()
@@ -473,8 +635,15 @@
     return launch_pred<true>(st, S, taps, bd, maxw, maxh, dst, sd, ref, sr, (const int32_t *)jobs, n);
 }
 
+static int pred_fuse()
+{
+    static const int mask = getenv("HAVOC_PRED_FUSE") ? atoi(getenv("HAVOC_PRED_FUSE")) & 3 : 3;
+    return mask;
+}
+
 template <bool BI>
-static hipError_t launch_pred_classes_t(hipStream_t st, int S, int taps, int bd, void *dst, long sd, const void *ref, long sr, const int32_t *j, const int count[4])
+static hipError_t launch_pred_classes_t(hipStream_t st, int S, int taps, int bd, void *dst, long sd, const void *ref, long sr, const int32_t *j, const int count[4],
+                                        const PredFollow *f = nullptr)
 {
     PredClasses pc;
     static const int jpw[4] = {32, 8, 2, 1};
@@ -489,12 +658,44 @@
     char *d = (char *)dst;
     const char *r = (const char *)ref;
     const dim3 g(pc.firstWg[4]), b(256);
+    if (f && (pred_fuse() & (BI ? 2 : 1)))
+    {
+        if (S == 1 && taps == 8) hipLaunchKernelGGL((k_pred_classes_fused<1, 8, BI>), g, b, 0, st, d, sd, r, sr, j, pc, bd, pred_lean(), *f);
+        else if (S == 1 && taps == 4) hipLaunchKernelGGL((k_pred_classes_fused<1, 4, BI>), g, b, 0, st, d, sd, r, sr, j, pc, bd, pred_lean(), *f);
+        else if (S == 2 && taps == 8) hipLaunchKernelGGL((k_pred_classes_fused<2, 8, BI>), g, b, 0, st, d, sd, r, sr, j, pc, bd, pred_lean(), *f);
+        else if (S == 2 && taps == 4) hipLaunchKernelGGL((k_pred_classes_fused<2, 4, BI>), g, b, 0, st, d, sd, r, sr, j, pc, bd, pred_lean(), *f);
+        else return hipErrorInvalidValue;
+        return hipGetLastError();
+    }
     if (S == 1 && taps == 8) hipLaunchKernelGGL((k_pred_classes<1, 8, BI>), g, b, 0, st, d, sd, r, sr, j, pc, bd, pred_lean());
     else if (S == 1 && taps == 4) hipLaunchKernelGGL((k_pred_classes<1, 4, BI>), g, b, 0, st, d, sd, r, sr, j, pc, bd, pred_lean());
     else if (S == 2 && taps == 8) hipLaunchKernelGGL((k_pred_classes<2, 8, BI>), g, b, 0, st, d, sd, r, sr, j, pc, bd, pred_lean());
     else if (S == 2 && taps == 4) hipLaunchKernelGGL((k_pred_classes<2, 4, BI>), g, b, 0, st, d, sd, r, sr, j, pc, bd, pred_lean());
     else return hipErrorInvalidValue;
+    if (f)
+    {
+        const int n = count[0] + count[1] + count[2] + count[3];
+        const dim3 gf((n + 3) / 4);
+        if (BI && S == 1) hipLaunchKernelGGL((k_pred_follow_subtract<1>), gf, b, 0, st, f->sub, f->stride_sub, d, sd, f->src, f->stride_src, j, n, bd, pred_lean());
+        else if (BI) hipLaunchKernelGGL((k_pred_follow_subtract<2>), gf, b, 0, st, f->sub, f->stride_sub, d, sd, f->src, f->stride_src, j, n, bd, pred_lean());
+        else if (S == 1) hipLaunchKernelGGL((k_pred_follow_satd<1>), gf, b, 0, st, f->src, f->stride_src, d, sd, j, n, f->cost);
+        else hipLaunchKernelGGL((k_pred_follow_satd<2>), gf, b, 0, st, f->src, f->stride_src, d, sd, j, n, f->cost);
+    }
     return hipGetLastError();
+}
+
+hipError_t launch_pred_uni_satd_classes(hipStream_t st, int S, int taps, int bd, void *dst, long sd, const void *ref, long sr, const havoc_mi355x_pred_uni_job *jobs,
+                                        const int count[4], const void *src, long ss, int32_t *cost)
+{
+    const PredFollow f = {(const char *)src, ss, cost, nullptr, 0};
+    return launch_pred_classes_t<false>(st, S, taps, bd, dst, sd, ref, sr, (const int32_t *)jobs, count, &f);
+}
+
+hipError_t launch_pred_bi_subtract_classes(hipStream_t st, int S, int taps, int bd, void *dst, long sd, const void *ref, long sr, const havoc_mi355x_pred_bi_job *jobs,
+                                           const int count[4], const void *src, long ss, void *sub, long ssub)
+{
+    const PredFollow f = {(const char *)src, ss, nullptr, (char *)sub, ssub};
+    return launch_pred_classes_t<true>(st, S, taps, bd, dst, sd, ref, sr, (const int32_t *)jobs, count, &f);
 }
 
 hipError_t launch_pred_bi_classes(hipStream_t st, int S, int taps, int bd, void *dst, long sd, const void *ref, long sr, const havoc_mi355x_pred_bi_job *jobs, const int count[4])
diff --git a/turingcodec_amd/csrc/kernels_metric.hip b/turingcodec_amd/csrc/kernels_metric.hip
--- a/turingcodec_amd/csrc/kernels_metric.hip
+++ b/turingcodec_amd/csrc/kernels_metric.hip
@@ -1,5 +1,6 @@
 #include "common.h"
 #include "launch.h"
+#include "block_bodies.h"
 
 #include <cstdlib>
 
@@ -812,130 +813,15 @@
 }
 
 
-template <int S, int N>
-__device__ __forceinline__ void load_diff_row(const char *a, const char *b, int (&d)[N])
-{
-    if (S == 1)
-    {
-        if (N == 8)
-        {
-            const u32x2 va = ld8(a), vb = ld8(b);
-#pragma unroll
-            for (int x = 0; x < 4; ++x)
-            {
-                d[x] = (int)((va.x >> (8 * x)) & 0xff) - (int)((vb.x >> (8 * x)) & 0xff);
-                d[x + 4] = (int)((va.y >> (8 * x)) & 0xff) - (int)((vb.y >> (8 * x)) & 0xff);
-            }
-        }
-        else
-        {
-            const uint32_t va = ld4(a), vb = ld4(b);
-#pragma unroll
-            for (int x = 0; x < 4; ++x) d[x] = (int)((va >> (8 * x)) & 0xff) - (int)((vb >> (8 * x)) & 0xff);
-        }
-    }
-    else
-    {
-        if (N == 8)
-        {
-            const u32x4 va = ld16(a), vb = ld16(b);
-            const uint32_t wa[4] = {va.x, va.y, va.z, va.w}, wb[4] = {vb.x, vb.y, vb.z, vb.w};
-#pragma unroll
-            for (int x = 0; x < 4; ++x)
-            {
-                d[2 * x] = (int)(wa[x] & 0xffff) - (int)(wb[x] & 0xffff);
-                d[2 * x + 1] = (int)(wa[x] >> 16) - (int)(wb[x] >> 16);
-            }
-        }
-        else
-        {
-            const u32x2 va = ld8(a), vb = ld8(b);
-            d[0] = (int)(va.x & 0xffff) - (int)(vb.x & 0xffff);
-            d[1] = (int)(va.x >> 16) - (int)(vb.x >> 16);
-            d[2] = (int)(va.y & 0xffff) - (int)(vb.y & 0xffff);
-            d[3] = (int)(va.y >> 16) - (int)(vb.y >> 16);
-        }
-    }
-}
-
 template <int S, int G>
 __global__ __launch_bounds__(256) void k_satd(const char *__restrict__ pa, long stride_a, const char *__restrict__ pb, long stride_b,
                                               const int32_t *__restrict__ jobs, int njobs, int32_t *__restrict__ out)
 {
-    typedef typename Sample<S>::T T;
     const int job = (xcd_block(blockIdx.x, gridDim.x) * 256 + threadIdx.x) / G;
     const int l = threadIdx.x & (G - 1);
     const bool live = job < njobs;
     const int32_t *j = jobs + (long)(live ? job : 0) * 4;
-    const int w = j[2], h = live ? j[3] : 0;
-    const long sab = stride_a * S, sbb = stride_b * S;
-    const char *a = pa + (long)j[0] * S;
-    const char *b = pb + (long)j[1] * S;
-    int acc = 0;
-    if (((w | h) & 7) == 0)
-    {
-        const int tw = w >> 3;
-        const FastDiv fd(tw);
-        for (int it = l; it < tw * (h >> 3) * 8; it += G)
-        {
-            const int tile = it >> 3, r = it & 7;
-            const int ty = fd.div(tile), tx = tile - ty * tw;
-            const char *pa8 = a + (long)(ty * 8 + r) * sab + tx * 8 * S, *pb8 = b + (long)(ty * 8 + r) * sbb + tx * 8 * S;
-            if (S == 1)
-            {
-                const u32x2 va = ld8(pa8), vb = ld8(pb8);
-                const uint32_t m = 0x00ff00ffu;
-                uint32_t p[4] = {pk_sub(va.x & m, vb.x & m), pk_sub((va.x >> 8) & m, (vb.x >> 8) & m),
-                                 pk_sub(va.y & m, vb.y & m), pk_sub((va.y >> 8) & m, (vb.y >> 8) & m)};
-                acc += satd_rows_pk<8>(p, r);
-            }
-            else
-            {
-                int d[8];
-                load_diff_row<S, 8>(pa8, pb8, d);
-                acc += satd_rows<S, 8>(d, r);
-            }
-        }
-    }
-    else if (((w | h) & 3) == 0)
-    {
-        const int tw = w >> 2;
-        const FastDiv fd(tw);
-        for (int it = l; it < tw * (h >> 2) * 4; it += G)
-        {
-            const int tile = it >> 2, r = it & 3;
-            const int ty = fd.div(tile), tx = tile - ty * tw;
-            const char *pa4 = a + (long)(ty * 4 + r) * sab + tx * 4 * S, *pb4 = b + (long)(ty * 4 + r) * sbb + tx * 4 * S;
-            if (S == 1)
-            {
-                const uint32_t va = ld4(pa4), vb = ld4(pb4), m = 0x00ff00ffu;
-                uint32_t p[2] = {pk_sub(va & m, vb & m), pk_sub((va >> 8) & m, (vb >> 8) & m)};
-                acc += satd_rows_pk<4>(p, r);
-            }
-            else
-            {
-                int d[4];
-                load_diff_row<S, 4>(pa4, pb4, d);
-                acc += satd_rows<S, 4>(d, r);
-            }
-        }
-    }
-    else
-    {
-        const int tw = w >> 1;
-        const FastDiv fd(tw);
-        for (int t = l; t < tw * (h >> 1); t += G)
-        {
-            const int ty = fd.div(t), tx = t - ty * tw;
-            const T *p = reinterpret_cast<const T *>(a + (long)(2 * ty) * sab) + 2 * tx;
-            const T *q = reinterpret_cast<const T *>(b + (long)(2 * ty) * sbb) + 2 * tx;
-            const int d0 = (int)p[0] - (int)q[0], d1 = (int)p[1] - (int)q[1];
-            const int d2 = (int)p[stride_a] - (int)q[stride_b], d3 = (int)p[stride_a + 1] - (int)q[stride_b + 1];
-            int sum = abs(d0 + d1 + d2 + d3) + abs(d0 - d1 + d2 - d3) + abs(d0 + d1 - d2 - d3) + abs(d0 - d1 - d2 + d3);
-            if (S == 2) sum >>= 2;
-            acc += sum;
-        }
-    }
+    const int acc = satd_block_share<S, G>(pa + (long)j[0] * S, stride_a, pb + (long)j[1] * S, stride_b, j[2], live ? j[3] : 0, l);
     const int t = G == 64 ? wave_sum(acc) : group_sum<G>(acc);
     if (live && l == 0) out[job] = t;
 }
diff --git a/turingcodec_amd/csrc/launch.h b/turingcodec_amd/csrc/launch.h
--- a/turingcodec_amd/csrc/launch.h
+++ b/turingcodec_amd/csrc/launch.h
@@ -19,6 +19,10 @@
 hipError_t launch_pred_bi(hipStream_t, int S, int taps, int bd, int maxw, int maxh, void *, long, const void *, long, const havoc_mi355x_pred_bi_job *, int);
 hipError_t launch_pred_uni_classes(hipStream_t, int S, int taps, int bd, void *, long, const void *, long, const havoc_mi355x_pred_uni_job *, const int count[4]);
 hipError_t launch_pred_bi_classes(hipStream_t, int S, int taps, int bd, void *, long, const void *, long, const havoc_mi355x_pred_bi_job *, const int count[4]);
+hipError_t launch_pred_uni_satd_classes(hipStream_t, int S, int taps, int bd, void *, long, const void *, long, const havoc_mi355x_pred_uni_job *, const int count[4],
+                                        const void *src, long stride_src, int32_t *cost);
+hipError_t launch_pred_bi_subtract_classes(hipStream_t, int S, int taps, int bd, void *, long, const void *, long, const havoc_mi355x_pred_bi_job *, const int count[4],
+                                           const void *src, long stride_src, void *sub, long stride_sub);
 hipError_t launch_subtract_bi(hipStream_t, int S, int bd, void *, long, const void *, long, const void *, long, const havoc_mi355x_subtract_bi_job *, int);
 hipError_t launch_subpel_satd(hipStream_t, int S, int taps, int bd, int maxw, int maxh, const void *, long, const void *, long, const havoc_mi355x_pred_uni_job *, int,
                               int32_t *);
diff --git a/turingcodec_amd/havoc.py b/turingcodec_amd/havoc.py
--- a/turingcodec_amd/havoc.py
+++ b/turingcodec_amd/havoc.py
@@ -78,6 +78,8 @@
         "subtract_bi": [_vp, _i, _i, _vp, _ip, _vp, _ip, _vp, _ip, _vp, _i],
         "pred_uni_classes": [_vp, _i, _i, _i, _vp, _ip, _vp, _ip, _vp, C.POINTER(C.c_int32)],
         "pred_bi_classes": [_vp, _i, _i, _i, _vp, _ip, _vp, _ip, _vp, C.POINTER(C.c_int32)],
+        "pred_uni_satd_classes": [_vp, _i, _i, _i, _vp, _ip, _vp, _ip, _vp, C.POINTER(C.c_int32), _vp, _ip, _vp],
+        "pred_bi_subtract_classes": [_vp, _i, _i, _i, _vp, _ip, _vp, _ip, _vp, C.POINTER(C.c_int32), _vp, _ip, _vp, _ip],
         "intra": [_vp, _i, _i, _i, _vp, _ip, _vp, _vp, _i],
         "intra_satd35": [_vp, _i, _i, _i, _vp, _ip, _vp, _vp, _i, _vp],
         "subpel_satd": [_vp, _i, _i, _i, _i, _i, _vp, _ip, _vp, _ip, _vp, _i, _vp],
@@ -610,6 +612,14 @@
         f = self.L.havoc_mi355x_pred_bi_classes if bi else self.L.havoc_mi355x_pred_uni_classes
         self._ck(f(self.h, self._S(ref), taps, bd, _ptr(dst), sd, _ptr(ref), sr, _ptr(jobs), c))
 
+    def pred_uni_satd_classes_d(self, taps, bd, dst, sd, ref, sr, jobs, counts, src, ss, cost):
+        c = (C.c_int32 * 4)(*[int(v) for v in counts])
+        self._ck(self.L.havoc_mi355x_pred_uni_satd_classes(self.h, self._S(ref), taps, bd, _ptr(dst), sd, _ptr(ref), sr, _ptr(jobs), c, _ptr(src), ss, _ptr(cost)))
+
+    def pred_bi_subtract_classes_d(self, taps, bd, dst, sd, ref, sr, jobs, counts, src, ss, sub, ssub):
+        c = (C.c_int32 * 4)(*[int(v) for v in counts])
+        self._ck(self.L.havoc_mi355x_pred_bi_subtract_classes(self.h, self._S(ref), taps, bd, _ptr(dst), sd, _ptr(ref), sr, _ptr(jobs), c, _ptr(src), ss, _ptr(sub), ssub))
+
     @staticmethod
     def size_classes(w, h):
         big = np.maximum(np.asarray(w), np.asarray(h))
diff --git a/turingcodec_amd/step.py b/turingcodec_amd/step.py
--- a/turingcodec_amd/step.py
+++ b/turingcodec_amd/step.py
@@ -1,4 +1,14 @@
 import numpy as np
+
+
+def followed_rows(jobs, wcol, pred_stride, followers, fol_pred, fol_w, fol_pred_stride):
+    jobs, fol = np.asarray(jobs), np.asarray(followers)
+    if pred_stride != fol_pred_stride or not len(jobs) or not len(fol) or len(np.unique(jobs[:, 0])) != len(jobs):
+        return None
+    order = np.argsort(jobs[:, 0], kind="stable")
+    row = order[np.minimum(np.searchsorted(jobs[order, 0], fol[:, fol_pred]), len(jobs) - 1)]
+    same = (jobs[row, 0] == fol[:, fol_pred]) & (jobs[row, wcol] == fol[:, fol_w]) & (jobs[row, wcol + 1] == fol[:, fol_w + 1])
+    return row if same.all() and len(np.unique(row)) == len(row) else None
 
 
 class DeviceFrame:
@@ -146,12 +156,27 @@
             def merged(name, jobs, wcol, bi, taps, dst, sd, ref, sr):
                 srt, counts, _ = hv.sort_by_class(np.asarray(jobs), np.asarray(jobs)[:, wcol], np.asarray(jobs)[:, wcol + 1])
                 return (name, lambda j=hv.up(srt), c=counts: hv.pred_classes_d(bi, taps, bd, dst, sd, ref, sr, j, c))
-            chain(merged("pred_uni8", wl.uni8, 2, False, 8, self.pred, 64, self.luma, st),
-                  ("satd_inter", lambda: hv.satd_d(self.luma, st, self.pred, 64, self.j_satd, self.o_satd)))
+            row = None if self.skip & {"pred_uni8", "satd_inter"} else followed_rows(wl.uni8, 2, 64, wl.satd_inter, 1, 2, 64)
+            if row is not None:
+                j = np.array(wl.uni8, np.int32)
+                j[row, 6] = np.asarray(wl.satd_inter)[:, 0]
+                j[row, 7] = 1 + np.arange(len(row))
+                srt, counts, _ = hv.sort_by_class(j, j[:, 2], j[:, 3])
+                chain(("pred_uni8", lambda j=hv.up(srt), c=counts: hv.pred_uni_satd_classes_d(8, bd, self.pred, 64, self.luma, st, j, c, self.luma, st, self.o_satd)))
+            else:
+                chain(merged("pred_uni8", wl.uni8, 2, False, 8, self.pred, 64, self.luma, st),
+                      ("satd_inter", lambda: hv.satd_d(self.luma, st, self.pred, 64, self.j_satd, self.o_satd)))
             chain(merged("pred_uni4", wl.uni4, 2, False, 4, self.cpred, 32, self.chroma, cst))
-            chain(merged("pred_bi8", wl.bi8, 3, True, 8, self.bi, 64, self.luma, st),
-                  ("subtract_bi", lambda: hv.subtract_bi_d(bd, self.sbi, 64, self.bi, 64, self.luma, st, self.j_sbi)),
-                  merged("pred_bi4", wl.bi4, 3, True, 4, self.cbi, 32, self.chroma, cst))
+            row = None if self.skip & {"pred_bi8", "subtract_bi"} else followed_rows(wl.bi8, 3, 64, wl.subtract_bi, 1, 3, 64)
+            if row is not None:
+                j = np.array(wl.bi8, np.int32)
+                j[row, 9], j[row, 10], j[row, 11] = np.asarray(wl.subtract_bi)[:, 2], np.asarray(wl.subtract_bi)[:, 0], 1
+                srt, counts, _ = hv.sort_by_class(j, j[:, 3], j[:, 4])
+                bi8 = [("pred_bi8", lambda j=hv.up(srt), c=counts: hv.pred_bi_subtract_classes_d(8, bd, self.bi, 64, self.luma, st, j, c, self.luma, st, self.sbi, 64))]
+            else:
+                bi8 = [merged("pred_bi8", wl.bi8, 3, True, 8, self.bi, 64, self.luma, st),
+                       ("subtract_bi", lambda: hv.subtract_bi_d(bd, self.sbi, 64, self.bi, 64, self.luma, st, self.j_sbi))]
+            chain(*bi8, merged("pred_bi4", wl.bi4, 3, True, 4, self.cbi, 32, self.chroma, cst))
         elif inter:
             chain(*classes("pred_uni8", wl.uni8, 2, lambda j, mw, mh: hv.pred_uni_d(8, bd, self.pred, 64, self.luma, st, j, mw, mh)),
                   ("satd_inter", lambda: hv.satd_d(self.luma, st, self.pred, 64, self.j_satd, self.o_satd)))
```

Measured after the change: 1591 frames/s, median of 6. Within noise of the previous version (+1.1%).
